# CIawevy/FreeFine

Measured on AMD Instinct MI355X. Metric: edited images/sec/GPU @512px 50-step DDIM, higher is better.
Workload: dtype bf16x3

## Files before the change

freefine_amd/_lib.py:

```python
import ctypes as C
import os

_HERE = os.path.dirname(os.path.abspath(__file__))
LIB_PATH = os.environ.get("FREEFINE_HIP_LIB") or os.path.join(_HERE, "libfreefine_hip.so")

FFN_F32, FFN_BF16, FFN_BF16X3, FFN_FP8 = 0, 1, 2, 3
IG_OUT_SILU, IG_OUT_F32, IG_GEGLU, IG_OUT_TRANSPOSED, IG_OUT_PAIR, IG_OUT_GELU, IG_OUT_RELU, IG_OUT_KV64 = 1, 2, 4, 8, 16, 32, 64, 128
IG_OUT_QGELU = 256
ELT_RELU, ELT_ADD, ELT_GELU = 0, 1, 2
ATT_MAXP, ATT_MAXB = 4, 16
ATT_HEAD_RULE, ATT_UNIFORM_SEL1, ATT_UNIFORM_SEL0, ATT_CAUSAL = 1, 2, 4, 8
NORM_SILU, NORM_OUT_PAIR = 1, 2
IMGPREP_MAX_SIDE = 4096
IMGPREP_MAX_TAPS = 2 * 3 * IMGPREP_MAX_SIDE + 1
BOX_NMS_MAX = 16384
KEEP_NONE, KEEP_SUM_LT128, KEEP_GT128 = 0, 1, 2


class IgemmDesc(C.Structure):
    _fields_ = [
        ("A", C.c_void_p), ("W", C.c_void_p), ("out", C.c_void_p),
        ("bias", C.c_void_p), ("rowbias", C.c_void_p), ("residual", C.c_void_p),
        ("M", C.c_int), ("N", C.c_int), ("K", C.c_int), ("Kpad", C.c_int),
        ("lda", C.c_int), ("ldo", C.c_int), ("ldr", C.c_int), ("ldrb", C.c_int),
        ("rows_per_batch", C.c_int),
        ("Hin", C.c_int), ("Win", C.c_int), ("Cin", C.c_int), ("Hout", C.c_int), ("Wout", C.c_int),
        ("stride", C.c_int), ("pad", C.c_int), ("upsample", C.c_int),
        ("flags", C.c_int), ("alpha", C.c_float), ("conv", C.c_int),
        ("splitk", C.c_int), ("ws", C.c_void_p), ("ws_bytes", C.c_long),
        ("a_lo", C.c_int), ("x3", C.c_int), ("f8", C.c_int), ("kv64_from", C.c_int),
    ]


class AttnEntry(C.Structure):
    _fields_ = [
        ("q_row", C.c_int), ("kv_row", C.c_int),
        ("w_const", C.c_float), ("w_slope", C.c_float),
        ("wq", C.c_void_p), ("kmask", C.c_void_p), ("qsel", C.c_void_p),
        ("flags", C.c_int), ("hr_row", C.c_int),
    ]


class AttnDesc(C.Structure):
    _fields_ = [
        ("q", C.c_void_p), ("k", C.c_void_p), ("vt", C.c_void_p), ("out", C.c_void_p), ("w_dev", C.c_void_p),
        ("Bo", C.c_int), ("S", C.c_int), ("Sk", C.c_int), ("heads", C.c_int), ("D", C.c_int),
        ("ldq", C.c_int), ("ldk", C.c_int), ("ldvt", C.c_int), ("ldo", C.c_int),
        ("scale", C.c_float), ("npass", C.c_int), ("out_pair", C.c_int), ("kv_pair", C.c_int),
        ("e", AttnEntry * (ATT_MAXP * ATT_MAXB)),
    ]


class CtrlStepDesc(C.Structure):
    _fields_ = [
        ("eps", C.c_void_p), ("x", C.c_void_p), ("noise", C.c_void_p), ("m", C.c_void_p), ("om", C.c_void_p),
        ("x_prev", C.c_void_p), ("pred_x0", C.c_void_p),
        ("c_bt", C.c_float), ("c_at", C.c_float), ("c_ap", C.c_float), ("c_dir", C.c_float),
        ("c_dirm", C.c_float * 8), ("stdv", C.c_float * 8), ("row_masked", C.c_int * 8),
        ("rows", C.c_int), ("CHW", C.c_int), ("HW", C.c_int),
    ]


class SplatXform(C.Structure):
    _fields_ = [("center", C.c_float * 3), ("translate", C.c_float * 3), ("rotate", C.c_float * 9), ("scale", C.c_float * 3),
                ("tan_half_fov", C.c_float)]


class PackDesc(C.Structure):
    _fields_ = [
        ("src", C.c_void_p), ("dst", C.c_void_p), ("src_row", C.c_int * 16),
        ("B", C.c_int), ("Cl", C.c_int), ("CP", C.c_int), ("HW", C.c_int),
    ]


class DiftDesc(C.Structure):
    _fields_ = [
        ("src", C.c_void_p), ("tgt", C.c_void_p), ("kps", C.c_void_p), ("ws", C.c_void_p), ("out_rc", C.c_void_p), ("out_cos", C.c_void_p),
        ("ws_bytes", C.c_long), ("es", C.c_long),
        ("dtype", C.c_int), ("E", C.c_int), ("C", C.c_int), ("ld", C.c_int), ("h", C.c_int), ("w", C.c_int), ("H", C.c_int), ("W", C.c_int), ("K", C.c_int),
    ]


class ResizePilDesc(C.Structure):
    _fields_ = [
        ("src", C.c_void_p), ("dst", C.c_void_p), ("scratch", C.c_void_p), ("m1", C.c_void_p), ("m2", C.c_void_p),
        ("hbounds", C.c_void_p), ("hcoef", C.c_void_p), ("vbounds", C.c_void_p), ("vcoef", C.c_void_p),
        ("B", C.c_int), ("H", C.c_int), ("W", C.c_int), ("C", C.c_int), ("oh", C.c_int), ("ow", C.c_int), ("hksize", C.c_int), ("vksize", C.c_int),
        ("y0", C.c_int), ("x0", C.c_int), ("ch", C.c_int), ("cw", C.c_int), ("rule", C.c_int),
    ]


class CoarseEditDesc(C.Structure):
    _fields_ = [
        ("src_img", C.c_void_p), ("src_mask", C.c_void_p), ("bg", C.c_void_p), ("hole_img", C.c_void_p), ("hole_mask", C.c_void_p), ("inv", C.c_void_p),
        ("final_img", C.c_void_p), ("tmask", C.c_void_p), ("trans_hole", C.c_void_p),
        ("B", C.c_int), ("H", C.c_int), ("W", C.c_int), ("mask_c", C.c_int), ("hole_mask_c", C.c_int),
    ]


_vp, _i, _f, _l = C.c_void_p, C.c_int, C.c_float, C.c_long
SYMBOLS = {
    "ffn_version": (_i, []),
    "ffn_last_error": (C.c_char_p, []),
    "ffn_device_info": (_i, [_i, C.c_char_p, _i]),
    "ffn_graph_launch": (_i, [_vp, _vp]),
    "ffn_igemm": (_i, [_vp, _i, C.POINTER(IgemmDesc)]),
    "ffn_conv3x3_n4": (_i, [_vp, _i, _vp, _vp, _vp, _vp, _i, _i, _i, _i]),
    "ffn_split_pair": (_i, [_vp, _vp, _vp, _l, _i, _i]),
    "ffn_groupnorm_f8": (_i, [_vp, _vp, _vp, _vp, _vp, _i, _i, _i, _i, _i, _f, _i, _f, _vp, _vp, _vp]),
    "ffn_attn": (_i, [_vp, _i, C.POINTER(AttnDesc)]),
    "ffn_attn_kernel_name": (_i, [_i, C.POINTER(AttnDesc), C.c_char_p, _i]),
    "ffn_igemm_tune": (_i, [_vp, _i, C.POINTER(IgemmDesc)]),
    "ffn_igemm_tune_entry_ints": (_i, []),
    "ffn_igemm_tune_export": (_i, [C.POINTER(C.c_int), _i]),
    "ffn_igemm_tune_import": (_i, [C.POINTER(C.c_int), _i]),
    "ffn_igemm_tune_stamp": (_i, []),
    "ffn_igemm_tune_clear": (_i, []),
    "ffn_igemm_tune_enable": (_i, [_i]),
    "ffn_igemm_num_configs": (_i, []),
    "ffn_igemm_force_config": (_i, [_i]),
    "ffn_igemm_kernel_name": (_i, [_i, C.POINTER(IgemmDesc), C.c_char_p, _i]),
    "ffn_attn_presplit": (_i, [_vp, _vp, _vp, _vp, _vp, _i, _i, _i, _i, _i]),
    "ffn_attn_variant": (_i, [_i, _i, C.POINTER(C.c_int), C.POINTER(C.c_int)]),
    "ffn_gn_nchunk": (_i, [_i]),
    "ffn_gn_fused": (_i, [_i, _i, _i, _i]),
    "ffn_gn_stats": (_i, [_vp, _i, _vp, _vp, _vp, _i, _i, _i, _i, _f, _vp, _vp, _vp]),
    "ffn_gn_apply": (_i, [_vp, _i, _vp, _vp, _vp, _vp, _i, _i, _i, _i]),
    "ffn_groupnorm": (_i, [_vp, _i, _vp, _vp, _vp, _vp, _i, _i, _i, _i, _f, _i, _vp, _vp, _vp]),
    "ffn_groupnorm_pair_raw": (_i, [_vp, _vp, _vp, _vp, _vp, _vp, _i, _i, _i, _i, _f, _i, _vp, _vp, _vp]),
    "ffn_layernorm": (_i, [_vp, _i, _vp, _vp, _vp, _vp, _i, _i, _f]),
    "ffn_layernorm_pair": (_i, [_vp, _vp, _vp, _vp, _vp, _i, _i, _f]),
    "ffn_softmax_rows": (_i, [_vp, _i, _vp, _vp, _l, _i, _f]),
    "ffn_pool_layernorm": (_i, [_vp, _i, _vp, _vp, _vp, _vp, _vp, _i, _i, _i, _f, _i]),
    "ffn_cosine_rows": (_i, [_vp, _vp, _vp, _vp, _i, _i, _i]),
    "ffn_cfg_masked": (_i, [_vp, _vp, _vp, _vp, _f, _vp, _l, _i]),
    "ffn_ddim_inv_step": (_i, [_vp, _vp, _vp, _f, _f, _f, _f, _vp, _vp, _l]),
    "ffn_ddim_ctrl_step": (_i, [_vp, C.POINTER(CtrlStepDesc)]),
    "ffn_pack_nchw": (_i, [_vp, _i, C.POINTER(PackDesc)]),
    "ffn_nhwc_to_nchw_f32": (_i, [_vp, _vp, _vp, _i, _i, _i, _i]),
    "ffn_concat": (_i, [_vp, _i, _vp, _vp, _vp, _l, _i, _i]),
    "ffn_timestep_embed": (_i, [_vp, _i, _vp, _vp, _vp, _i, _i, _i]),
    "ffn_transpose": (_i, [_vp, _i, _vp, _vp, _i, _i, _i, _i, _i]),
    "ffn_cast": (_i, [_vp, _i, _i, _vp, _vp, _l]),
    "ffn_eltwise": (_i, [_vp, _i, _i, _vp, _vp, _vp, _l]),
    "ffn_resize_bilinear": (_i, [_vp, _i, _vp, _vp, _i, _i, _i, _i, _i, _i, _i]),
    "ffn_splat_lift": (_i, [_vp, _vp, _vp, _vp, _i, _i, _i, _f, _f]),
    "ffn_splat_project": (_i, [_vp, _vp, _vp, _i, C.POINTER(SplatXform)]),
    "ffn_splat_bin": (_i, [_vp, _i, _vp, _i, _f, _i, _i, _vp, _vp, _vp]),
    "ffn_splat_render": (_i, [_vp, _vp, _vp, _vp, _vp, _f, _i, _i, _i, _vp, _vp, _vp]),
    "ffn_splat_ids": (_i, [_vp, _vp, _vp, _vp, _f, _i, _i, _i, _vp]),
    "ffn_splat_correspond": (_i, [_vp, _vp, _vp, _i, _i, _i, _vp, _i, _vp, _vp]),
    "ffn_geo_project": (_i, [_vp, _vp, C.POINTER(C.c_float), _f, _i, _i, _vp, _vp]),
    "ffn_splat_composite": (_i, [_vp, _vp, _vp, _vp, _vp, _f, _f, _i, _i, _i, _i, _i, _vp]),
    "ffn_mesh_cover": (_i, [_vp, _vp, _vp, _i, _i, _vp]),
    "ffn_embed_tokens": (_i, [_vp, _i, _vp, _vp, _vp, _vp, _l, _i, _i, _i]),
    "ffn_dift_match": (_i, [_vp, C.POINTER(DiftDesc)]),
    "ffn_dift_workspace_bytes": (_l, [_i, _i, _i, _i]),
    "ffn_sift_base": (_i, [_vp, _vp, _vp, _i, _i, _i]),
    "ffn_gauss_blur_f32": (_i, [_vp, _vp, _vp, _vp, _i, _i, _vp, _i]),
    "ffn_decimate2_f32": (_i, [_vp, _vp, _vp, _i, _i]),
    "ffn_sift_extrema": (_i, [_vp, _vp, _vp, _i, _i, _vp, _i, _vp, C.POINTER(C.c_int)]),
    "ffn_sift_refine_orient": (_i, [_vp, _vp, _vp, _i, _i, _i, _vp, _i, _vp]),
    "ffn_sift_describe": (_i, [_vp, _vp, _i, _i, _i, _vp, _i, _vp, _vp]),
    "ffn_knn2_u8": (_i, [_vp, _vp, _i, _vp, _i, _vp, _vp]),
    "ffn_resize_pil_bilinear_u8": (_i, [_vp, _vp, _vp, _vp, _i, _i, _i, _i, _i, _vp, _vp, _i, _vp, _vp, _i]),
    "ffn_resize_pil_u8": (_i, [_vp, C.POINTER(ResizePilDesc)]),
    "ffn_resize_taps8_u8": (_i, [_vp, _vp, _vp, _i, _i, _i, _i, _i, _i, _vp, _vp, _vp, _vp]),
    "ffn_resize_gather_u8": (_i, [_vp, _vp, _vp, _i, _i, _i, _i, _i, _i, _vp, _vp, _i]),
    "ffn_dilate_u8": (_i, [_vp, _vp, _vp, _vp, _i, _i, _i, _i, _i]),
    "ffn_mask_bbox_u8": (_i, [_vp, _vp, _vp, _i, _i, _i, _i]),
    "ffn_coarse_edit_2d": (_i, [_vp, C.POINTER(CoarseEditDesc)]),
    "ffn_vit_patch_rows": (_i, [_vp, _i, _vp, _vp, _vp, _i, _i, _i, _i, _i]),
    "ffn_vit_patch_rows_pair": (_i, [_vp, _vp, _vp, _vp, _i, _i, _i, _i, _i]),
    "ffn_sam_patch_rows": (_i, [_vp, _i, _vp, _vp, _i, _i, _i, _i, _i, _i, C.POINTER(C.c_float), C.POINTER(C.c_float)]),
    "ffn_sam_patch_rows_pair": (_i, [_vp, _vp, _vp, _i, _i, _i, _i, _i, _i, C.POINTER(C.c_float), C.POINTER(C.c_float)]),
    "ffn_hyper_masks": (_i, [_vp, _vp, _vp, _vp, _i, _i, _i, _i]),
    "ffn_upsample_bicubic": (_i, [_vp, _vp, _vp, _vp, _i, _i, _i, _i, _i]),
    "ffn_upsample_bicubic_stats": (_i, [_vp, _vp, _vp, _vp, _i, _i, _i, _i, _i, _f]),
    "ffn_box_nms": (_i, [_vp, _vp, _vp, _i, _f]),
    "ffn_image_to_nhwc": (_i, [_vp, _i, _vp, _vp, _l, _i]),
    "ffn_nhwc_to_image": (_i, [_vp, _i, _vp, _vp, _i, _i, _i]),
}

_lib = None


class FreeFineHipError(RuntimeError):
    pass


def load():
    global _lib
    if _lib is None:
        if not os.path.exists(LIB_PATH):
            raise FreeFineHipError(
                f"{LIB_PATH} not found: build it with `python -c 'import __graft_entry__ as g; g.build()'` "
                "(hipcc --offload-arch=gfx950). There is no CPU fallback for the product path.")
        import torch
        lib = C.CDLL(LIB_PATH)
        for name, (res, args) in SYMBOLS.items():
            fn = getattr(lib, name)
            fn.restype = res
            fn.argtypes = args
        _lib = lib
    return _lib


def check(rc, what=""):
    if rc != 0:
        msg = load().ffn_last_error()
        raise FreeFineHipError(f"{what} failed rc={rc}: {msg.decode() if msg else ''}")
```

freefine_amd/csrc/capi.hip:

```cpp
#include <hip/hip_runtime.h>
#include <stdarg.h>
#include <stdio.h>
#include <initializer_list>
#include <mutex>
#include <unordered_map>
#include <stdlib.h>
#include <string.h>

#include "../../include/freefine_hip.h"
#include "attention.h"
#include "attention_pp.h"
#include "attention_x.h"
#include "attention_x3.h"
#include "attention_x3p.h"
#include "attention_xx3.h"
#include "conv_small.h"
#include "elementwise.h"
#include "igemm.h"
#include "igemm_p8.h"
#include "norms.h"
#include "splat.h"

static thread_local char g_err[512] = "";
static int fail(int code, const char* fmt, ...) {
    va_list ap;
    va_start(ap, fmt);
    vsnprintf(g_err, sizeof(g_err), fmt, ap);
    va_end(ap);
    return code;
}
static int check_launch(const char* what) {
    hipError_t e = hipGetLastError();
    if (e != hipSuccess) return fail(FFN_EHIP, "%s: %s", what, hipGetErrorString(e));
    return FFN_OK;
}
#define LAUNCH(...)                  \
    do {                             \
        (void)hipGetLastError();     \
        hipLaunchKernelGGL(__VA_ARGS__); \
    } while (0)
#define REQUIRE(cond, ...) \
    do {                   \
        if (!(cond)) return fail(FFN_EINVAL, __VA_ARGS__); \
    } while (0)

static inline bool aligned16(const void* p) { return (reinterpret_cast<uintptr_t>(p) & 15) == 0; }
static inline int grid_for(long n, int per_block = 256, int cap = 4096) {
    long g = (n + per_block - 1) / per_block;
    if (g < 1) g = 1;
    if (g > cap) g = cap;
    return (int)g;
}

template <typename K>
static int set_lds(K kernel, int bytes) {
    static std::mutex mu;
    static std::unordered_map<const void*, int> done;
    if (bytes > 48 * 1024) {
        std::lock_guard<std::mutex> lk(mu);
        int& have = done[reinterpret_cast<const void*>(kernel)];
        if (have >= bytes) return FFN_OK;
        have = bytes;
        hipError_t e = hipFuncSetAttribute(reinterpret_cast<const void*>(kernel), hipFuncAttributeMaxDynamicSharedMemorySize, bytes);
        if (e != hipSuccess) return fail(FFN_EHIP, "hipFuncSetAttribute(%d): %s", bytes, hipGetErrorString(e));
    }
    return FFN_OK;
}

extern "C" int ffn_version(void) { return 14; }
extern "C" const char* ffn_last_error(void) { return g_err; }
extern "C" int ffn_device_info(int device, char* name, int name_len) {
    hipDeviceProp_t prop;
    hipError_t e = hipGetDeviceProperties(&prop, device);
    if (e != hipSuccess) return fail(FFN_EHIP, "hipGetDeviceProperties: %s", hipGetErrorString(e));
    if (name && name_len > 0) {
        strncpy(name, prop.gcnArchName, name_len - 1);
        name[name_len - 1] = 0;
    }
    return prop.multiProcessorCount;
}

extern "C" int ffn_graph_launch(void* stream, void* graph_exec) {
    REQUIRE(graph_exec, "graph_launch: null graph");
    hipError_t e = hipGraphLaunch(reinterpret_cast<hipGraphExec_t>(graph_exec), reinterpret_cast<hipStream_t>(stream));
    if (e != hipSuccess) return fail(FFN_EHIP, "hipGraphLaunch: %s", hipGetErrorString(e));
    return FFN_OK;
}

static int device_cus() {
    static const int n = [] {
        int dev = 0, v = 0;
        if (hipGetDevice(&dev) != hipSuccess || hipDeviceGetAttribute(&v, hipDeviceAttributeMultiprocessorCount, dev) != hipSuccess || v <= 0) v = 256;
        return v;
    }();
    return n;
}
static bool can_split(const ffn_igemm_desc& d) {
    return d.ws && d.splitk != 1 && !(d.flags & (FFN_IG_GEGLU | FFN_IG_OUT_TRANSPOSED | FFN_IG_OUT_KV64));
}
static void igemm_rule_for(int dtype, const ffn_igemm_desc& d, int* bm, int* bn, int* splitk) {
    const long t128 = (long)((d.M + 127) / 128) * ((d.N + 127) / 128);
    const long t12864 = (long)((d.M + 127) / 128) * ((d.N + 63) / 64);
    *splitk = 1;
    if (!d.conv && !(d.flags & FFN_IG_GEGLU) && d.M >= 128 && (!can_split(d) || t12864 >= 128)) {
        *bm = 128; *bn = 64;
    } else if (d.N > 64 && (t128 >= 256 || (can_split(d) && d.M > 512 && d.N >= 128))) {
        *bm = 128; *bn = 128;
    } else if (t12864 >= 256 || d.M >= 4096 || (can_split(d) && d.M >= 96 && d.N >= 64)) {
        *bm = 128; *bn = 64;
    } else { *bm = 64; *bn = 64; }
    if (can_split(d)) {
        const int kstage = dtype == FFN_F32 ? 32 : 64;
        const int nk = (d.K + kstage - 1) / kstage;
        const long tiles = (long)((d.M + *bm - 1) / *bm) * ((d.N + *bn - 1) / *bn);
        int s = d.splitk > 1 ? d.splitk : (tiles >= 224 ? 1 : (int)((448 + tiles - 1) / tiles));
        if (d.splitk <= 1 && s > nk / 6) s = nk / 6;
        const long per = (long)d.M * d.N * 4;
        if ((long)s * per > d.ws_bytes) s = (int)(d.ws_bytes / per);
        if (s > nk) s = nk;
        if (s < 1) s = 1;
        *splitk = s;
    }
}

enum { CFG_64x64, CFG_128x64, CFG_128x128_8, CFG_128x128_16, CFG_256x128, CFG_256x256, CFG_128x320, CFG_128x160, CFG_192x320, CFG_H_128x320, CFG_H_256x128, CFG_H_256x256, CFG_H_128x128, CFG_PP_256x320, CFG_PP_256x256, CFG_PP_192x320, CFG_PP_192x256, CFG_PP_256x128, CFG_COUNT };
struct IgCfgInfo { int bm, bn, nwm, nwn; };
static const IgCfgInfo kCfg[CFG_COUNT] = {{64, 64, 2, 2}, {128, 64, 4, 2}, {128, 128, 2, 4}, {128, 128, 4, 4},
                                          {256, 128, 4, 4}, {256, 256, 4, 4}, {128, 320, 4, 4}, {128, 160, 4, 2}, {192, 320, 3, 4},
                                          {128, 320, 4, 4}, {256, 128, 4, 4}, {256, 256, 4, 4}, {128, 128, 4, 4},
                                          {256, 320, 2, 4}, {256, 256, 2, 4}, {192, 320, 2, 4}, {192, 256, 2, 4},
                                          {256, 128, 2, 4}};
struct IgChoice { int cfg, splitk; };
struct TunedEntry { IgChoice ch; bool validated; };

static bool is_halo_cfg(int cfg) { return cfg == CFG_H_128x320 || cfg == CFG_H_256x128 || cfg == CFG_H_256x256 || cfg == CFG_H_128x128; }
static bool is_pp_cfg(int cfg) { return cfg >= CFG_PP_256x320 && cfg <= CFG_PP_256x128; }
static bool pp_ok(const ffn_igemm_desc& d, int bm, int bn, int splitk = 1) {
    const long lim = (1l << 31) - 4096;
    const int nkt = d.x3 ? d.K / 96 : d.K / 64;
    if (bn == 128 && (bm != 256 || !d.x3 || d.conv != 1 || splitk > 1 || d.N % 256 == 0 || d.N % 320 == 0 || (d.flags & (FFN_IG_GEGLU | FFN_IG_OUT_PAIR | FFN_IG_OUT_KV64 | FFN_IG_OUT_TRANSPOSED)))) return false;
    if (d.x3) {
        if (d.x3 != 2 || d.K % 96 != 0 || d.a_lo != 32) return false;
    } else if (d.K % 64 != 0) return false;
    if (nkt < 2 || d.N % bn != 0 || d.M < bm) return false;
    const int osz = d.x3 ? 4 : 2;
    if (splitk > 1) {
        if (!can_split(d) || nkt % splitk != 0 || nkt / splitk < 2 || (long)splitk * d.M * d.N * 4 > d.ws_bytes || (long)splitk * d.M * d.N * 4 >= lim) return false;
    } else {
        const int act_ok = (!d.residual && !d.x3 && !d.f8 && !(d.flags & FFN_IG_GEGLU)) ? (FFN_IG_OUT_GELU | FFN_IG_OUT_RELU) : 0;
        if ((d.alpha != 1.0f && !d.f8) || (d.flags & ~(FFN_IG_GEGLU | act_ok | (d.x3 ? (FFN_IG_OUT_F32 | FFN_IG_OUT_PAIR | FFN_IG_OUT_KV64) : 0)))) return false;
        if (d.f8 && (!d.conv || (d.flags & FFN_IG_GEGLU))) return false;
        if (d.x3 && (d.flags & FFN_IG_GEGLU) && !(d.flags & FFN_IG_OUT_PAIR)) return false;
        if ((d.flags & FFN_IG_OUT_PAIR) && !(d.flags & FFN_IG_GEGLU) && (d.N % 32 != 0 || (d.ldo / 2) % 32 != 0 || (d.flags & FFN_IG_OUT_TRANSPOSED))) return false;
        if ((d.flags & FFN_IG_GEGLU) && bn != 256) return false;
        if (d.rowbias && d.rows_per_batch < 128) return false;
    }
    long a_bytes;
    if (d.conv) {
        const int pix = d.x3 ? d.lda : d.Cin;
        const int cpt = d.x3 ? d.Cin / 32 : d.Cin / 64;
        if (d.Cin % (d.x3 ? 32 : 64) != 0 || d.K != (d.conv == 2 ? 4 : 9) * (d.x3 ? 3 : 1) * d.Cin) return false;
        if (d.x3 && d.lda != 2 * d.Cin) return false;
        if (d.conv == 2 && (d.f8 || d.stride != 1 || d.upsample)) return false;
        if ((long)cpt * 9 * cpt >= 65536) return false;
        a_bytes = (long)(d.M / (d.Hout * d.Wout)) * d.Hin * d.Win * pix * 2;
        if (2 * d.Hin + 2 >= 32768 || 2 * d.Win + 2 >= 32768) return false;
        if (a_bytes + 256l * pix * 2 >= lim) return false;
    } else {
        a_bytes = (long)d.M * d.lda * 2;
        if (a_bytes + 256l * d.lda * 2 >= lim) return false;
    }
    if ((long)d.N * d.Kpad * 2 >= lim || (long)(d.M + 256) * d.ldo * ((d.flags & FFN_IG_OUT_PAIR) ? 2 : osz) >= lim) return false;
    if (d.residual && (long)(d.M + 256) * d.ldr * osz >= lim) return false;
    return true;
}
static int halo_bytes_for(const ffn_igemm_desc& d, int bm) {
    if (!d.conv || d.stride != 1 || d.upsample || d.pad != 1 || d.Hin != d.Hout || d.Win != d.Wout) return 0;
    if (d.Cin % 64 != 0 || d.Cin > 30000 || d.K != 9 * d.Cin || d.M % bm != 0) return 0;
    const int H = d.Hin, W = d.Win;
    int tw, tr;
    if (W <= bm) {
        if (bm % W != 0 || (H * W) % bm != 0) return 0;
        tw = W; tr = bm / W;
    } else {
        if (W % bm != 0) return 0;
        tw = bm; tr = 1;
    }
    const int nq = ((tr + 2) * (tw + 2) + 7) / 8;
    if (nq > 4 * 16) return 0;
    return nq * 8 * 128;
}
static bool x3_cfg(int cfg) { return cfg == CFG_64x64 || cfg == CFG_128x64 || cfg == CFG_128x128_8 || is_pp_cfg(cfg); }
static ffn_igemm_desc x3_view(const ffn_igemm_desc& d) {
    ffn_igemm_desc v = d;
    v.x3 = d.x3 == 2 ? 2 : 1;
    v.f8 = 0;
    v.K = 3 * d.K;
    v.flags |= FFN_IG_OUT_F32;
    return v;
}
static ffn_igemm_desc f8_view(const ffn_igemm_desc& d) {
    ffn_igemm_desc v = d;
    v.f8 = 1;
    v.x3 = 0;
    v.K = d.K / 2;
    v.Cin = d.Cin / 2;
    v.Kpad = d.Kpad / 2;
    v.lda = d.lda / 2;
    return v;
}
static ffn_igemm_desc igemm_view(int dtype, const ffn_igemm_desc& d) {
    if (dtype == FFN_BF16X3) return x3_view(d);
    if (dtype == FFN_FP8) return f8_view(d);
    ffn_igemm_desc v = d;
    v.x3 = v.f8 = 0;
    return v;
}
static int pp_tile_height(const ffn_igemm_desc& d, int bn, std::initializer_list<int> heights, int min_fill4, bool trans = false) {
    long best = -1;
    int bh = 0;
    for (int h : heights) {
        if (trans ? d.M < h : !pp_ok(d, h, bn)) continue;
        const long tiles = (long)((d.M + h - 1) / h) * (d.N / bn);
        if (tiles * 4 < (long)device_cus() * min_fill4) continue;
        const long cost = ((tiles + device_cus() - 1) / device_cus()) * h;
        if (best < 0 || cost < best) { best = cost; bh = h; }
    }
    return bh;
}
static int pp_cfg(int bm, int bn) {
    for (int cfg = CFG_PP_256x320; cfg <= CFG_PP_256x128; ++cfg)
        if (kCfg[cfg].bm == bm && kCfg[cfg].bn == bn) return cfg;
    return -1;
}
static bool conv2_tile(const ffn_igemm_desc& d, int* bm, int* bn) {
    for (int n : {320, 256})
        for (int h : {256, 192})
            if (pp_tile_height(d, n, {h}, 0)) { *bm = h; *bn = n; return true; }
    return false;
}
static bool pp_trans_tile(const ffn_igemm_desc& d, int* bm, int* bn) {
    const long lim = (1l << 31) - 4096;
    *bn = d.N % 320 == 0 ? 320 : (d.N % 256 == 0 ? 256 : 0);
    if (!*bn || d.alpha != 1.0f || d.rows_per_batch % 16 != 0 || d.M % 4 != 0) return false;
    if (d.x3) {
        if (d.x3 != 2 || d.K % 96 != 0 || d.K < 192 || d.a_lo != 32) return false;
    } else if (d.K % 64 != 0 || d.K < 128) return false;
    if ((long)(d.M + 256) * d.lda * 2 >= lim || (long)d.N * d.Kpad * 2 >= lim) return false;
    if ((long)((d.M + d.rows_per_batch - 1) / d.rows_per_batch) * d.N * d.ldo * (d.x3 ? 4 : 2) >= lim) return false;
    return (*bm = pp_tile_height(d, *bn, {256, 192}, 0, true)) != 0;
}
static IgChoice rule_choice(int dtype, const ffn_igemm_desc& d) {
    int bm, bn, sk;
    igemm_rule_for(dtype, d, &bm, &bn, &sk);
    const int kstage = dtype == FFN_F32 ? 32 : 64;
// ... 65 lines not shown
            const int hb = halo_bytes_for(d, c.bm);
            if (hb <= 0 || d.splitk > 1 || 2 * hb + 2 * c.bn * 128 > 160 * 1024) continue;
            if ((cfg == CFG_H_128x320) && (d.flags & FFN_IG_GEGLU)) continue;
        }
        const bool halo = is_halo_cfg(cfg) || is_pp_cfg(cfg);
        if (is_pp_cfg(cfg)) {
            const long pt = (long)((d.M + c.bm - 1) / c.bm) * (d.N / (c.bn > 0 ? c.bn : 1));
            if (d.splitk <= 1 && pp_ok(d, c.bm, c.bn) && n < cap) out[n++] = IgChoice{cfg, 1};
            if (cfg != CFG_PP_256x128 && d.splitk != 1 && pt > 0 && pt < kPpSplitBelow && d.N % c.bn == 0) {
                const int nkt = d.x3 ? d.K / 96 : d.K / 64;
                int added = 0;
                for (int sgo = (int)((384 + pt - 1) / pt); sgo >= 2 && added < 2; --sgo) {
                    if (d.splitk > 1 && sgo != d.splitk) continue;
                    if (nkt % sgo != 0 || nkt / sgo < 2 || !pp_ok(d, c.bm, c.bn, sgo)) continue;
                    if (n < cap) out[n++] = IgChoice{cfg, sgo};
                    ++added;
                }
            }
            continue;
        }
        if (c.bm > 64 && c.bm >= 2 * d.M) continue;
        if (c.bn > 64 && c.bn >= 2 * d.N) continue;
        if (cfg == CFG_64x64 && (long)d.M * d.N > (1l << 22)) continue;
        const long tiles = (long)((d.M + c.bm - 1) / c.bm) * ((d.N + c.bn - 1) / c.bn);
        int splits[3] = {1, 0, 0};
        if (d.splitk > 1) {
            int sf = (can_split(d) && !halo) ? d.splitk : 1;
            if ((long)sf * per > d.ws_bytes) sf = (int)(d.ws_bytes / per);
            if (sf > nk) sf = nk;
            splits[0] = sf >= 2 ? sf : 1;
        } else if (can_split(d) && !halo) {
            for (int t = 0; t < 2; ++t) {
                int sgo = (int)(((t ? 512 : 256) + tiles / 2) / tiles);
                if (sgo > nk / 4) sgo = nk / 4;
                if ((long)sgo * per > d.ws_bytes) sgo = (int)(d.ws_bytes / per);
                if (sgo >= 2) splits[1 + t] = sgo;
            }
            if (splits[2] == splits[1]) splits[2] = 0;
        }
        for (int t = 0; t < 3 && n < cap; ++t) {
            if (!splits[t]) continue;
            bool dup = false;
            for (int j = 0; j < n; ++j) dup |= out[j].cfg == cfg && out[j].splitk == splits[t];
            if (!dup) out[n++] = IgChoice{cfg, splits[t]};
        }
    }
    return n;
}
static int g_force_cfg = -1;
extern "C" int ffn_igemm_num_configs(void) { return CFG_COUNT; }
extern "C" int ffn_igemm_force_config(int cfg) {
    const int prev = g_force_cfg;
    g_force_cfg = (cfg >= 0 && cfg < CFG_COUNT) ? cfg : -1;
    return prev;
}
static bool known_choice(const ffn_igemm_desc& d, IgChoice* ch) {
    IgChoice cand[40];
    if (g_force_cfg >= 0) {
        *ch = heuristic_choice(d);
        for (int i = candidates_for(d, cand, 40) - 1; i >= 0; --i)
            if (cand[i].cfg == g_force_cfg) *ch = cand[i];
        return true;
    }
    std::lock_guard<std::mutex> lk(g_tune_mu);
    auto it = g_tuned.find(tune_key(d));
    if (it == g_tuned.end()) return false;
    if (!it->second.validated) {
        const int nc = candidates_for(d, cand, 40);
        bool ok = false;
        for (int i = 0; i < nc; ++i) ok |= cand[i].cfg == it->second.ch.cfg && cand[i].splitk == it->second.ch.splitk;
        if (!ok) return g_tuned.erase(it), false;
        it->second.validated = true;
    }
    *ch = it->second.ch;
    return true;
}

enum IgKind { IG_RING, IG_HALO, IG_PP, IG_PP_TRANS };
struct IgemmPlan {
    IgKind kind;
    bool f32;
    int bm, bn, amode, nwm, nwn;
    bool swap, fastk, x3, f8;
    bool res, geglu, split;
    int splitk, halo_bytes, lds;
    bool reduce_f32;
    dim3 grid, block;
};
static int igemm_plan(int dtype, const ffn_igemm_desc& d, const IgChoice* ch, IgemmPlan* p) {
    *p = IgemmPlan{};
    p->f32 = dtype == FFN_F32;
    p->x3 = d.x3 != 0;
    p->f8 = d.f8 != 0;
    p->amode = d.conv ? AMODE_CONV3 : AMODE_DENSE;
    p->swap = !(d.flags & FFN_IG_OUT_TRANSPOSED);
    p->reduce_f32 = p->f32 || p->x3;
    p->splitk = 1;
    p->block = dim3(512);
    const bool tuned = ch != nullptr;
    IgChoice rule;
    if (!tuned && !p->f32 && pp_trans_tile(d, &p->bm, &p->bn)) {
        p->kind = IG_PP_TRANS;
    } else {
        if (!tuned) ch = &(rule = rule_choice(p->f32 ? FFN_F32 : FFN_BF16, d));
        REQUIRE(ch->cfg >= 0 && ch->cfg < CFG_COUNT, "igemm: bad configuration %d", ch->cfg);
        REQUIRE(!(p->x3 || p->f8) || x3_cfg(ch->cfg), "igemm: configuration %d is not built for split-bf16 / fp8 problems", ch->cfg);
        const IgCfgInfo& c = kCfg[ch->cfg];
        p->kind = is_halo_cfg(ch->cfg) ? IG_HALO : (is_pp_cfg(ch->cfg) ? IG_PP : IG_RING);
        p->bm = c.bm; p->bn = c.bn; p->nwm = c.nwm; p->nwn = c.nwn;
        p->splitk = ch->splitk;
        p->block = dim3(64 * c.nwm * c.nwn);
        if (!tuned && p->x3) p->nwm = p->nwn = 2, p->block = dim3(256);
    }
    const int ntm = (d.M + p->bm - 1) / p->bm, ntn = (d.N + p->bn - 1) / p->bn;
    switch (p->kind) {
    case IG_RING: {
        p->fastk = tuned && !p->x3 && !p->f8 && (d.conv ? d.Cin % 64 == 0 : d.K % 64 == 0) && (long)d.K * 2 + 256 <= (long)sizeof(g_zero_page);
        p->lds = 2 * (p->bm + p->bn) * 128;
        int gx = ntm * ntn;
        if (tuned || p->x3) {
            int per_cu = (160 * 1024) / p->lds;
            if (per_cu > 2048 / (int)p->block.x) per_cu = 2048 / (int)p->block.x;
            const int cap = (device_cus() * per_cu) / p->splitk;
            if (gx > cap && cap >= 8) gx = cap;
        }
        p->grid = dim3(gx, p->splitk);
        break;
    }
    case IG_HALO:
        p->halo_bytes = halo_bytes_for(d, p->bm);
        REQUIRE(p->halo_bytes > 0 && p->splitk == 1 && !p->x3 && !p->f8, "igemm: halo kernel not applicable");
        p->lds = 2 * p->halo_bytes + 2 * p->bn * 128;
        p->grid = dim3((d.M / p->bm) * ntn);
        break;
    case IG_PP:
        REQUIRE(pp_ok(d, p->bm, p->bn, p->splitk), "igemm: ping-pong kernel not applicable");
        p->split = p->splitk > 1;
        p->res = !p->split && d.residual;
        p->geglu = !p->split && !d.conv && (d.flags & FFN_IG_GEGLU);
        [[fallthrough]];
    case IG_PP_TRANS: {
        p->lds = 2 * (p->bm + p->bn) * 128 + 12288;
        const int nt = ntm * (d.N / p->bn) * p->splitk;
        p->grid = dim3(nt < device_cus() ? nt : device_cus());
        break;
    }
    }
    return FFN_OK;
}
template <typename K, typename... A>
static int igemm_launch(const IgemmPlan& p, K kern, hipStream_t s, A... args) {
    static const char* const what[] = {"igemm", "igemm(halo)", "igemm(ping-pong)", "igemm(ping-pong, transposed)"};
    if (int rc = set_lds(kern, p.lds)) return rc;
    LAUNCH(kern, p.grid, p.block, p.lds, s, args...);
    return check_launch(what[p.kind]);
}
template <typename T, int AMODE, bool SWAP, bool FASTK = false, bool X3 = false, bool F8 = false>
static int launch_ring(const IgemmPlan& p, hipStream_t s, const ffn_igemm_desc& d) {
#define FFN_RING(BM_, BN_, WM_, WN_) \
    if (p.bm == BM_ && p.bn == BN_ && p.nwm == WM_ && p.nwn == WN_) return igemm_launch(p, igemm_glds_kernel<T, BM_, BN_, AMODE, SWAP, 2, WM_, WN_, FASTK, X3, F8>, s, d)
    if constexpr (X3 && !SWAP) {
        FFN_RING(64, 64, 2, 2);
        FFN_RING(128, 64, 2, 2);
        FFN_RING(128, 128, 2, 2);
    } else {
        FFN_RING(64, 64, 2, 2);
        FFN_RING(128, 64, 4, 2);
        FFN_RING(128, 128, 2, 4);
        if constexpr (!X3 && !F8) FFN_RING(128, 128, 4, 4);
        if constexpr (sizeof(T) == 2 && SWAP && !X3 && !F8) {
            FFN_RING(256, 128, 4, 4);
            FFN_RING(256, 256, 4, 4);
            FFN_RING(128, 320, 4, 4);
            FFN_RING(128, 160, 4, 2);
            FFN_RING(192, 320, 3, 4);
        }
    }
#undef FFN_RING
    return fail(FFN_EINVAL, "igemm: no %d x %d tile on %d x %d waves for this problem", p.bm, p.bn, p.nwm, p.nwn);
}
template <int AMODE, bool X3 = false, bool F8 = false>
static int launch_pp(const IgemmPlan& p, hipStream_t s, const ffn_igemm_desc& d) {
    const bool trans = p.kind == IG_PP_TRANS;
#define FFN_PP(BM_, BN_, RES_, GEGLU_, SPLIT_, TRANS_)                                                                       \
    if (p.bm == BM_ && p.bn == BN_ && p.res == RES_ && p.geglu == GEGLU_ && p.split == SPLIT_ && trans == TRANS_) \
        return igemm_launch(p, igemm_pp_kernel<BM_, BN_, AMODE, RES_, GEGLU_, SPLIT_, TRANS_, X3, F8>, s, d, p.splitk)
#define FFN_PP_TILE(BM_, BN_)                                                                   \
    FFN_PP(BM_, BN_, false, false, false, false);                                               \
    FFN_PP(BM_, BN_, true, false, false, false);                                                \
    FFN_PP(BM_, BN_, false, false, true, false);                                                \
    if constexpr (AMODE == AMODE_DENSE && !F8) {                                                \
        FFN_PP(BM_, BN_, false, false, false, true);                                            \
        if constexpr (BN_ == 256) FFN_PP(BM_, BN_, false, true, false, false);                  \
    }
    FFN_PP_TILE(256, 320)
    FFN_PP_TILE(256, 256)
    FFN_PP_TILE(192, 320)
    FFN_PP_TILE(192, 256)
    if constexpr (X3 && AMODE == AMODE_CONV3) {
        FFN_PP(256, 128, false, false, false, false);
        FFN_PP(256, 128, true, false, false, false);
    }
#undef FFN_PP_TILE
#undef FFN_PP
    return fail(FFN_EINVAL, "igemm: no %d x %d ping-pong tile of this form", p.bm, p.bn);
}
static int igemm_run(hipStream_t s, int dtype, const ffn_igemm_desc& d, const IgChoice* ch) {
    IgemmPlan p;
    int rc = igemm_plan(dtype, d, ch, &p);
    if (rc) return rc;
    const bool conv = p.amode == AMODE_CONV3;
    switch (p.kind) {
    case IG_RING:
        if (p.f32) rc = conv ? launch_ring<float, AMODE_CONV3, true>(p, s, d) : (p.swap ? launch_ring<float, AMODE_DENSE, true>(p, s, d) : launch_ring<float, AMODE_DENSE, false>(p, s, d));
        else if (!p.swap) rc = p.x3 ? launch_ring<bf16, AMODE_DENSE, false, false, true>(p, s, d) : launch_ring<bf16, AMODE_DENSE, false>(p, s, d);
        else if (p.x3) rc = conv ? launch_ring<bf16, AMODE_CONV3, true, false, true>(p, s, d) : launch_ring<bf16, AMODE_DENSE, true, false, true>(p, s, d);
        else if (p.f8) rc = launch_ring<bf16, AMODE_CONV3, true, false, false, true>(p, s, d);
        else if (p.fastk) rc = conv ? launch_ring<bf16, AMODE_CONV3, true, true>(p, s, d) : launch_ring<bf16, AMODE_DENSE, true, true>(p, s, d);
        else rc = conv ? launch_ring<bf16, AMODE_CONV3, true>(p, s, d) : launch_ring<bf16, AMODE_DENSE, true>(p, s, d);
        break;
    case IG_HALO:
#define FFN_HALO(BM_, BN_) \
    if (p.bm == BM_ && p.bn == BN_) rc = igemm_launch(p, igemm_halo_kernel<bf16, BM_, BN_, 4, 4>, s, d, p.halo_bytes)
        FFN_HALO(128, 320);
        FFN_HALO(256, 128);
        FFN_HALO(256, 256);
        FFN_HALO(128, 128);
#undef FFN_HALO
        break;
    case IG_PP:
    case IG_PP_TRANS:
        if (p.x3) rc = conv ? launch_pp<AMODE_CONV3, true>(p, s, d) : launch_pp<AMODE_DENSE, true>(p, s, d);
        else if (p.f8) rc = launch_pp<AMODE_CONV3, false, true>(p, s, d);
        else rc = conv ? launch_pp<AMODE_CONV3>(p, s, d) : launch_pp<AMODE_DENSE>(p, s, d);
        break;
    }
    if (rc || p.splitk == 1) return rc;
    const dim3 grid(grid_for((long)d.M * (d.N / 4)));
    if (p.reduce_f32) LAUNCH(igemm_splitk_reduce_kernel<float>, grid, dim3(256), 0, s, d, p.splitk);
    else LAUNCH(igemm_splitk_reduce_kernel<bf16>, grid, dim3(256), 0, s, d, p.splitk);
    return check_launch("igemm_splitk_reduce");
}
static int igemm_tune_now(hipStream_t s, int dtype, const ffn_igemm_desc& d) {
    std::lock_guard<std::mutex> lk(g_tune_mu);
    IgChoice cand[40];
    const int nc = candidates_for(d, cand, 40);
    hipEvent_t e0, e1;
    if (hipEventCreate(&e0) != hipSuccess || hipEventCreate(&e1) != hipSuccess) return igemm_run(s, dtype, d, &cand[0]);
    IgChoice best = cand[0];
    float best_ms = 1e30f;
    const int reps = 3;
    for (int i = 0; i < nc; ++i) {
        int rc = igemm_run(s, dtype, d, &cand[i]);
        if (rc) continue;
        float ms = 1e30f;
        for (int round = 0; round < 2 && !rc; ++round) {
            (void)hipEventRecord(e0, s);
            for (int r = 0; r < reps && !rc; ++r) rc = igemm_run(s, dtype, d, &cand[i]);
            (void)hipEventRecord(e1, s);
            if (rc || hipEventSynchronize(e1) != hipSuccess) { rc = rc ? rc : FFN_EHIP; break; }
            float t = 0.f;
            (void)hipEventElapsedTime(&t, e0, e1);
            if (t < ms) ms = t;
        }
        if (rc) continue;
        if (ms < best_ms) { best_ms = ms; best = cand[i]; }
    }
    (void)hipEventDestroy(e0);
    (void)hipEventDestroy(e1);
    g_tuned[tune_key(d)] = TunedEntry{best, true};
    static const bool verbose = getenv("FFN_IGEMM_TUNE_VERBOSE") != nullptr;
    if (verbose)
        fprintf(stderr, "[ffn tune] %s M=%d N=%d K=%d flags=%d -> %dx%d split %d (%.1f us, %d candidates)\n", d.conv ? "conv" : "dense", d.M, d.N,
                d.K, d.flags, kCfg[best.cfg].bm, kCfg[best.cfg].bn, best.splitk, best_ms * 1e3f / reps, nc);
    return igemm_run(s, dtype, d, &best);
}
static constexpr int kTuneEntryInts = (int)(sizeof(TuneKey) / sizeof(int)) + 3;
static constexpr int kTuneStamp = 0x67780000 ^ (950 << 4) ^ ((int)sizeof(TuneKey) << 8) ^ CFG_COUNT ^ (4 << 24);
extern "C" int ffn_igemm_tune_entry_ints(void) { return kTuneEntryInts; }
extern "C" int ffn_igemm_tune_stamp(void) { return kTuneStamp; }
extern "C" int ffn_igemm_tune_clear(void) {
    std::lock_guard<std::mutex> lk(g_tune_mu);
    const int n = (int)g_tuned.size();
    g_tuned.clear();
    return n;
}
extern "C" int ffn_igemm_tune_enable(int on) {
    std::lock_guard<std::mutex> lk(g_tune_mu);
    const int prev = g_tune_runtime;
    g_tune_runtime = on ? 1 : 0;
    return prev;
}
extern "C" int ffn_igemm_tune_export(int* buf, int max_entries) {
    std::lock_guard<std::mutex> lk(g_tune_mu);
    int n = 0;
    for (const auto& kv : g_tuned) {
        if (buf && n < max_entries) {
            int* e = buf + (long)n * kTuneEntryInts;
            e[0] = kTuneStamp;
            memcpy(e + 1, &kv.first, sizeof(TuneKey));
            e[kTuneEntryInts - 2] = kv.second.ch.cfg;
            e[kTuneEntryInts - 1] = kv.second.ch.splitk;
        }
        ++n;
    }
    return n;
}
extern "C" int ffn_igemm_tune_import(const int* buf, int n_entries) {
    REQUIRE(buf || n_entries == 0, "igemm_tune_import: null buffer");
    std::lock_guard<std::mutex> lk(g_tune_mu);
    int n = 0;
    for (int i = 0; i < n_entries; ++i) {
        const int* e = buf + (long)i * kTuneEntryInts;
        if (e[0] != kTuneStamp) continue;
        TuneKey k;
        memcpy(&k, e + 1, sizeof(TuneKey));
        const IgChoice ch{e[kTuneEntryInts - 2], e[kTuneEntryInts - 1]};
        if (ch.cfg < 0 || ch.cfg >= CFG_COUNT || ch.splitk < 1) continue;
        g_tuned[k] = TunedEntry{ch, false};
        ++n;
    }
    return n;
}
static int igemm_validate(int dtype, const ffn_igemm_desc& d) {
    REQUIRE(dtype == FFN_F32 || dtype == FFN_BF16 || dtype == FFN_BF16X3 || dtype == FFN_FP8, "igemm: bad dtype %d", dtype);
    if (dtype == FFN_FP8) {
        REQUIRE(d.conv && d.Cin > 0 && d.Cin % 16 == 0 && d.K == 9 * d.Cin && d.Kpad >= d.K && d.Kpad % 16 == 0 && d.lda == d.Cin,
                "igemm(fp8): 3x3 convolutions with Cin %% 16 == 0 only (Cin=%d, K=%d, Kpad=%d, lda=%d)", d.Cin, d.K, d.Kpad, d.lda);
        REQUIRE(d.M > 0 && d.N > 0 && d.N % 4 == 0 && d.ldo % 4 == 0 && d.rows_per_batch > 0 && d.M % (d.Hout * d.Wout) == 0, "igemm(fp8): bad shape");
        REQUIRE(!(d.flags & (FFN_IG_GEGLU | FFN_IG_OUT_TRANSPOSED | FFN_IG_OUT_PAIR | FFN_IG_OUT_F32)), "igemm(fp8): plain / SiLU / residual epilogues only");
        REQUIRE(d.stride == 1 || d.stride == 2, "igemm(fp8): stride %d", d.stride);
        int ex = 0;
        REQUIRE(d.alpha > 0.f && frexpf(d.alpha, &ex) == 0.5f, "igemm(fp8): alpha must be a power of two (the un-scaling of two power-of-two operand scales)");
        if (d.residual) REQUIRE(d.ldr % 4 == 0 && d.ldr >= d.N, "igemm(fp8): ldr=%d must be a multiple of 4 and >= N=%d", d.ldr, d.N);
        REQUIRE(d.ldo >= d.N, "igemm(fp8): ldo=%d must be >= N=%d", d.ldo, d.N);
        return FFN_OK;
    }
    const int epc = dtype == FFN_F32 ? 4 : 8;
    const int kmul = dtype == FFN_BF16X3 ? (d.x3 == 2 ? 2 : 3) : 1;
    REQUIRE(d.M > 0 && d.N > 0 && d.K > 0, "igemm: empty problem M=%d N=%d K=%d", d.M, d.N, d.K);
    REQUIRE(d.Kpad >= kmul * d.K && d.Kpad % epc == 0, "igemm: Kpad=%d (row stride of W) must be >= %d x K=%d and a multiple of %d", d.Kpad, kmul, d.K, epc);
    if (dtype == FFN_BF16X3) {
        const int plane = d.conv ? d.Cin : d.K;
        if (d.x3 == 2) {
            REQUIRE(plane % 32 == 0 && d.a_lo == 32 && d.lda >= 2 * plane, "igemm: blocked split-bf16 operands need K (conv: Cin) %% 32 == 0, a_lo = 32, lda >= 2 x that (%d, a_lo=%d, lda=%d)", plane, d.a_lo, d.lda);
        } else {
            REQUIRE(d.a_lo % 8 == 0 && d.a_lo >= plane && d.a_lo + plane <= d.lda, "igemm: split-bf16 A needs planes of %d elements: a_lo=%d, lda=%d", plane, d.a_lo, d.lda);
        }
        REQUIRE(d.lda % 8 == 0, "igemm: lda=%d must be a multiple of 8", d.lda);
        REQUIRE(d.alpha == 1.0f, "igemm: split-bf16 problems take alpha = 1");
    }
    REQUIRE(d.K % epc == 0, "igemm: K=%d must be a multiple of %d", d.K, epc);
    REQUIRE(d.rows_per_batch > 0, "igemm: rows_per_batch must be > 0");
    if (d.conv) {
        REQUIRE(d.Cin % epc == 0, "igemm: Cin=%d must be a multiple of %d", d.Cin, epc);
        if (d.conv == 2) {
            REQUIRE((dtype == FFN_BF16 || dtype == FFN_BF16X3) && d.K == 4 * d.Cin && d.stride == 1 && d.upsample == 0 && d.pad >= 0 && d.pad <= 3 && d.splitk <= 1,
                    "igemm: 2x2 convolution needs FFN_BF16 / FFN_BF16X3, K = 4*Cin, stride 1, no upsample, pad in 0..3, no forced split");
            int bm, bn;
            REQUIRE(conv2_tile(igemm_view(dtype, d), &bm, &bn), "igemm: 2x2 convolution M=%d N=%d Cin=%d fits no ping-pong tile (Cin %% 64 (split-bf16: 32), N %% 256 / 320, M >= 192)", d.M, d.N, d.Cin);
        } else {
            REQUIRE(d.conv == 1, "igemm: conv=%d", d.conv);
            REQUIRE(d.K == 9 * d.Cin, "igemm: conv K=%d != 9*Cin=%d", d.K, 9 * d.Cin);
        }
        REQUIRE(d.stride == 1 || d.stride == 2, "igemm: stride %d", d.stride);
        REQUIRE(d.upsample == 0 || d.upsample == 1, "igemm: upsample %d", d.upsample);
        REQUIRE(d.M % (d.Hout * d.Wout) == 0, "igemm: M=%d not a multiple of Hout*Wout", d.M);
    } else {
        REQUIRE(d.lda % epc == 0, "igemm: lda=%d must be a multiple of %d", d.lda, epc);
    }
    if (d.flags & FFN_IG_OUT_KV64) {
        REQUIRE(dtype == FFN_BF16X3 && !d.conv && !d.residual && !d.rowbias && d.splitk <= 1 &&
                    !(d.flags & (FFN_IG_GEGLU | FFN_IG_OUT_PAIR | FFN_IG_OUT_SILU | FFN_IG_OUT_GELU | FFN_IG_OUT_RELU | FFN_IG_OUT_QGELU)),
                "igemm: FFN_IG_OUT_KV64 needs FFN_BF16X3, dense A, the plain epilogue and no forced split-K");
        if (d.flags & FFN_IG_OUT_TRANSPOSED) REQUIRE(d.rows_per_batch % 64 == 0 && d.M % d.rows_per_batch == 0 && d.ldo >= d.rows_per_batch && d.ldo % 64 == 0,
                                                     "igemm: KV64 transposed output needs rows_per_batch %% 64 == 0, whole batches, ldo %% 64 == 0 (rows_per_batch=%d, ldo=%d)", d.rows_per_batch, d.ldo);
        else REQUIRE(d.kv64_from >= 0 && d.kv64_from < d.N && d.kv64_from % 64 == 0 && d.N % 64 == 0 && d.ldo % 4 == 0,
                     "igemm: KV64 output needs kv64_from and N %% 64 == 0 (kv64_from=%d, N=%d)", d.kv64_from, d.N);
    }
    if (d.flags & FFN_IG_OUT_TRANSPOSED) {
        REQUIRE(!d.conv, "igemm: transposed output is only supported for dense A");
        REQUIRE(d.ldo % 4 == 0, "igemm: transposed ldo=%d must be a multiple of 4", d.ldo);
        REQUIRE(!(d.flags & (FFN_IG_GEGLU | FFN_IG_OUT_F32 | FFN_IG_OUT_SILU | FFN_IG_OUT_GELU | FFN_IG_OUT_RELU | FFN_IG_OUT_QGELU)) && !d.residual && !d.rowbias,
                "igemm: transposed output supports bias only");
    } else {
        REQUIRE(d.N % 4 == 0 && d.ldo % 4 == 0, "igemm: N=%d and ldo=%d must be multiples of 4", d.N, d.ldo);
        if (d.residual) REQUIRE(d.ldr % 4 == 0, "igemm: ldr=%d must be a multiple of 4", d.ldr);
        if (d.flags & FFN_IG_OUT_PAIR) {
            const int nout = (d.flags & FFN_IG_GEGLU) ? d.N / 2 : d.N;
            REQUIRE(dtype == FFN_BF16X3 && d.ldo % 16 == 0 && d.ldo / 2 >= nout, "igemm: pair output needs FFN_BF16X3, ldo %% 16 == 0, ldo/2 >= columns");
            REQUIRE(d.residual != d.out, "igemm: pair output cannot overwrite its fp32 residual");
            REQUIRE((d.ldo / 2) % 32 != 0 || nout % 32 == 0 || nout == d.ldo / 2, "igemm: blocked pair output (ldo/2 %% 32 == 0) needs whole 32-column blocks");
            REQUIRE(nout == d.ldo / 2 || (d.ldo / 2) % 32 == 0, "igemm: pair output into a wider row needs ldo/2 %% 32 == 0 (ldo=%d, columns=%d)", d.ldo, nout);
        }
        if (d.flags & FFN_IG_GEGLU) {
            REQUIRE(d.N % 64 == 0, "igemm: GEGLU needs N %% 64 == 0 (N=%d)", d.N);
            REQUIRE(!d.residual && !d.rowbias && !(d.flags & (FFN_IG_OUT_F32 | FFN_IG_OUT_SILU | FFN_IG_OUT_GELU | FFN_IG_OUT_RELU | FFN_IG_OUT_QGELU)), "igemm: GEGLU epilogue is exclusive");
        }
    }
    const int act = d.flags & (FFN_IG_OUT_SILU | FFN_IG_OUT_GELU | FFN_IG_OUT_RELU | FFN_IG_OUT_QGELU);
    REQUIRE((act & (act - 1)) == 0, "igemm: SILU / GELU / QGELU / RELU are mutually exclusive");
    REQUIRE(d.splitk >= 0, "igemm: splitk must be >= 0");
    if (!d.conv && dtype != FFN_BF16X3) REQUIRE(d.lda >= d.K, "igemm: lda=%d must be >= K=%d", d.lda, d.K);
    if (d.flags & FFN_IG_OUT_TRANSPOSED) {
        const int cols = d.rows_per_batch < d.M ? d.rows_per_batch : d.M;
        REQUIRE(d.ldo >= cols, "igemm: transposed ldo=%d must be >= the %d rows of a batch", d.ldo, cols);
    } else if (!(d.flags & FFN_IG_OUT_PAIR)) {
        const int nout = (d.flags & FFN_IG_GEGLU) ? d.N / 2 : d.N;
        REQUIRE(d.ldo >= nout, "igemm: ldo=%d must be >= the %d output columns", d.ldo, nout);
    }
    if (d.residual) REQUIRE(d.ldr >= d.N, "igemm: ldr=%d must be >= N=%d", d.ldr, d.N);
    return FFN_OK;
}
static bool tuned_family(int dtype, const ffn_igemm_desc& d) { return dtype != FFN_F32 && !(d.flags & FFN_IG_OUT_TRANSPOSED); }
extern "C" int ffn_igemm_kernel_name(int dtype, const ffn_igemm_desc* d0, char* buf, int len) {
    REQUIRE(d0 && buf && len > 0, "igemm_kernel_name: null argument");
    if (int rc = igemm_validate(dtype, *d0)) return rc;
    const ffn_igemm_desc d = igemm_view(dtype, *d0);
    const bool tuned = tuned_family(dtype, d);
    IgChoice ch;
    if (tuned && !known_choice(d, &ch)) ch = heuristic_choice(d);
    IgemmPlan p;
    if (int rc = igemm_plan(dtype, d, tuned ? &ch : nullptr, &p)) return rc;
    auto b = [](bool v) { return v ? "true" : "false"; };
    switch (p.kind) {
    case IG_RING:
        snprintf(buf, len, "void igemm_glds_kernel<%s, %d, %d, %d, %s, 2, %d, %d, %s, %s, %s>(ffn_igemm_desc)", p.f32 ? "float" : "bf16", p.bm, p.bn, p.amode,
                 b(p.swap), p.nwm, p.nwn, b(p.fastk), b(p.x3), b(p.f8));
        break;
    case IG_HALO: snprintf(buf, len, "void igemm_halo_kernel<bf16, %d, %d, %d, %d>(ffn_igemm_desc, int)", p.bm, p.bn, p.nwm, p.nwn); break;
    case IG_PP:
    case IG_PP_TRANS:
        snprintf(buf, len, "void igemm_pp_kernel<%d, %d, %d, %s, %s, %s, %s, %s, %s>(ffn_igemm_desc, int)", p.bm, p.bn, p.amode, b(p.res), b(p.geglu), b(p.split),
                 b(p.kind == IG_PP_TRANS), b(p.x3), b(p.f8));
        break;
    }
    return FFN_OK;
}
extern "C" int ffn_split_pair(void* stream, const float* src, void* dst, long rows, int C, int ld_src) {
    REQUIRE(src && dst && rows > 0 && C > 0 && C % 4 == 0 && ld_src >= C && ld_src % 4 == 0, "split_pair: bad arguments (C=%d, ld_src=%d)", C, ld_src);
    REQUIRE(aligned16(src) && aligned16(dst), "split_pair: pointers must be 16-byte aligned");
    static const int wide = [] { const char* e = getenv("FFN_PAIR8"); return e ? atoi(e) : 1; }();
    if (wide && C % 8 == 0 && ld_src % 4 == 0) LAUNCH(split_pair8_kernel, dim3(grid_for(rows * (C / 8))), dim3(256), 0, reinterpret_cast<hipStream_t>(stream), src, (bf16*)dst, rows, C, ld_src);
    else LAUNCH(split_pair_kernel, dim3(grid_for(rows * (C / 4))), dim3(256), 0, reinterpret_cast<hipStream_t>(stream), src, (bf16*)dst, rows, C, ld_src);
    return check_launch("split_pair");
}
extern "C" int ffn_conv3x3_n4(void* stream, int dtype, const void* x, const float* w, const float* bias, float* out, int B, int H, int W, int Cin) {
    REQUIRE(dtype == FFN_F32 || dtype == FFN_BF16, "conv3x3_n4: fp32 or bf16 activations");
    REQUIRE(x && w && out && aligned16(x) && aligned16(w) && aligned16(out) && (!bias || aligned16(bias)), "conv3x3_n4: null / unaligned pointer");
    REQUIRE(B > 0 && H > 0 && W > 0 && Cin > 0 && Cin % 16 == 0 && Cin <= 448, "conv3x3_n4: B=%d H=%d W=%d Cin=%d (Cin %% 16 == 0, <= 448)", B, H, W, Cin);
    hipStream_t s = reinterpret_cast<hipStream_t>(stream);
    const long npix = (long)B * H * W;
    const int lds = 36 * Cin * 4;
    dim3 grid((unsigned)((npix + 63) / 64));
    int rc;
    if (dtype == FFN_F32) {
        if ((rc = set_lds(conv3x3_n4_kernel<float>, lds))) return rc;
        LAUNCH(conv3x3_n4_kernel<float>, grid, dim3(256), lds, s, (const float*)x, w, bias, out, B, H, W, Cin);
    } else {
        if ((rc = set_lds(conv3x3_n4_kernel<bf16>, lds))) return rc;
        LAUNCH(conv3x3_n4_kernel<bf16>, grid, dim3(256), lds, s, (const bf16*)x, w, bias, out, B, H, W, Cin);
    }
    return check_launch("conv3x3_n4");
}
extern "C" int ffn_igemm(void* stream, int dtype, const ffn_igemm_desc* d0) {
    REQUIRE(d0, "igemm: null descriptor");
    if (int rc = igemm_validate(dtype, *d0)) return rc;
    if (dtype == FFN_FP8) {
        REQUIRE(d0->A && d0->W && d0->out && aligned16(d0->A) && aligned16(d0->W) && aligned16(d0->out), "igemm(fp8): A/W/out must be non-null and 16-byte aligned");
    } else {
        REQUIRE(d0->A && d0->W && d0->out, "igemm: null A/W/out");
        REQUIRE(aligned16(d0->A) && aligned16(d0->W) && aligned16(d0->out), "igemm: A/W/out must be 16-byte aligned");
    }
    if ((dtype == FFN_BF16X3 || dtype == FFN_F32) && d0->residual) REQUIRE(aligned16(d0->residual), "igemm: fp32 residual must be 16-byte aligned");
    if ((dtype == FFN_BF16 || dtype == FFN_FP8) && d0->residual)
        REQUIRE((reinterpret_cast<uintptr_t>(d0->residual) & 7) == 0, "igemm%s: bf16 residual must be 8-byte aligned", dtype == FFN_FP8 ? "(fp8)" : "");
    if (d0->ws) REQUIRE(aligned16(d0->ws) && d0->ws_bytes >= 0, "igemm%s: workspace must be 16-byte aligned", dtype == FFN_FP8 ? "(fp8)" : "");
    hipStream_t s = reinterpret_cast<hipStream_t>(stream);
    const ffn_igemm_desc d = igemm_view(dtype, *d0);
    if (!tuned_family(dtype, d)) return igemm_run(s, dtype, d, nullptr);
    IgChoice ch;
    if (!known_choice(d, &ch)) {
        hipStreamCaptureStatus cap = hipStreamCaptureStatusNone;
        (void)hipStreamIsCapturing(s, &cap);
        if (tune_enabled() && cap == hipStreamCaptureStatusNone && d.residual != d.out) return igemm_tune_now(s, dtype, d);
        ch = heuristic_choice(d);
    }
    return igemm_run(s, dtype, d, &ch);
}

extern "C" int ffn_igemm_tune(void* stream, int dtype, const ffn_igemm_desc* d) { return ffn_igemm(stream, dtype, d); }

struct AttnTile { int dp, qf, kt, occ; };
static const AttnTile kAttnTileF32[] = {{48, 2, 64, 1}, {64, 2, 64, 1}, {80, 2, 64, 1}, {160, 1, 32, 1}};
static const AttnTile kAttnTileBf16[] = {{64, 2, 64, 2}, {96, 2, 64, 1}, {160, 1, 64, 1}};
static AttnTile attn_tile(bool f32, int D) {
    const AttnTile* t = f32 ? kAttnTileF32 : kAttnTileBf16;
    const int n = f32 ? 4 : 3;
    int i = 0;
    while (i + 1 < n && D > t[i].dp) ++i;
    return t[i];
}
extern "C" int ffn_attn_variant(int dtype, int D, int* dp, int* qf) {
    REQUIRE(dp && qf, "attn_variant: null argument");
    const AttnTile t = attn_tile(dtype == FFN_F32, D);
    *dp = t.dp;
    *qf = t.qf;
    return FFN_OK;
}
static constexpr int attn_kernel_lds(int esz, int dp, int qf, int kt) {
    return 2 * (kt * (dp * esz == 128 ? 128 : dp * esz + 16) + dp * ((dp * esz == 128 && kt * esz == 128) ? 128 : kt * esz + 16)) + 4 * (dp / 16) * qf * 64 * 16 + 2 * kt;
}
static_assert(attn_kernel_lds(4, 160, 1, 32) <= 160 * 1024 && attn_kernel_lds(2, 160, 1, 64) <= 160 * 1024, "attention tile does not fit the 160 KiB LDS");

typedef void (*attn_x3w_t)(ffn_attn_desc);
extern "C" __attribute__((visibility("hidden"))) attn_x3w_t fx3w_kernel(int masks);
extern "C" __attribute__((visibility("hidden"))) int fx3w_lds_bytes(void);
// ... 699 lines not shown
    }
    return check_launch("gn_apply");
}
extern "C" int ffn_layernorm(void* stream, int dtype, const void* x, void* y, const float* gamma, const float* beta, int M, int C,
                             float eps) {
    REQUIRE(dtype == FFN_F32 || dtype == FFN_BF16, "layernorm: bad dtype");
    const int epc = dtype == FFN_F32 ? 4 : 8;
    REQUIRE(x && y && gamma && beta && C % epc == 0 && aligned16(x) && aligned16(y), "layernorm: bad arguments");
    const int cch = C / epc;
    REQUIRE(cch <= 64 * 6, "layernorm: C=%d too large", C);
    hipStream_t s = reinterpret_cast<hipStream_t>(stream);
    const int grid = (M + 3) / 4;
    if (dtype == FFN_F32) {
        if (cch <= 128) LAUNCH((layernorm_kernel<float, 2>), dim3(grid), dim3(256), 0, s, (const float*)x, (float*)y, gamma, beta, M, C, eps);
        else LAUNCH((layernorm_kernel<float, 6>), dim3(grid), dim3(256), 0, s, (const float*)x, (float*)y, gamma, beta, M, C, eps);
    } else {
        if (cch <= 128) LAUNCH((layernorm_kernel<bf16, 2>), dim3(grid), dim3(256), 0, s, (const bf16*)x, (bf16*)y, gamma, beta, M, C, eps);
        else LAUNCH((layernorm_kernel<bf16, 6>), dim3(grid), dim3(256), 0, s, (const bf16*)x, (bf16*)y, gamma, beta, M, C, eps);
    }
    return check_launch("layernorm");
}
extern "C" int ffn_layernorm_pair(void* stream, const float* x, void* y, const float* gamma, const float* beta, int M, int C, float eps) {
    REQUIRE(x && y && gamma && beta && C % 4 == 0 && aligned16(x) && aligned16(y), "layernorm_pair: bad arguments");
    const int cch = C / 4;
    REQUIRE(cch <= 64 * 6, "layernorm_pair: C=%d too large", C);
    hipStream_t s = reinterpret_cast<hipStream_t>(stream);
    const int grid = (M + 3) / 4;
    if (cch <= 128) LAUNCH((layernorm_kernel<float, 2, true>), dim3(grid), dim3(256), 0, s, x, (float*)y, gamma, beta, M, C, eps);
    else LAUNCH((layernorm_kernel<float, 6, true>), dim3(grid), dim3(256), 0, s, x, (float*)y, gamma, beta, M, C, eps);
    return check_launch("layernorm(pair)");
}
extern "C" int ffn_softmax_rows(void* stream, int dtype, const void* x, void* y, long M, int N, float scale) {
    REQUIRE(dtype == FFN_F32 || dtype == FFN_BF16, "softmax_rows: bad dtype");
    REQUIRE(x && y && M > 0 && N > 0, "softmax_rows: bad arguments");
    hipStream_t s = reinterpret_cast<hipStream_t>(stream);
    if (dtype == FFN_F32) LAUNCH(softmax_rows_kernel<float>, dim3((unsigned)M), dim3(256), 0, s, (const float*)x, (float*)y, N, scale);
    else LAUNCH(softmax_rows_kernel<bf16>, dim3((unsigned)M), dim3(256), 0, s, (const bf16*)x, (bf16*)y, N, scale);
    return check_launch("softmax_rows");
}

extern "C" int ffn_cfg_masked(void* stream, const float* eps_u, const float* eps_c, const float* mask, float cfg, float* eps, long n,
                              int HW) {
    REQUIRE(eps_u && eps_c && eps && n > 0 && HW > 0, "cfg_masked: bad arguments");
    LAUNCH(cfg_masked_kernel, dim3(grid_for(n)), dim3(256), 0, reinterpret_cast<hipStream_t>(stream), eps_u, eps_c, mask, cfg, eps, n, HW);
    return check_launch("cfg_masked");
}
extern "C" int ffn_ddim_inv_step(void* stream, const float* eps, const float* x, float c_bt, float c_at, float c_an, float c_bn,
                                 float* x_next, float* pred_x0, long n) {
    REQUIRE(eps && x && x_next && n > 0, "ddim_inv_step: bad arguments");
    LAUNCH(ddim_inv_step_kernel, dim3(grid_for(n)), dim3(256), 0, reinterpret_cast<hipStream_t>(stream), eps, x, c_bt, c_at, c_an, c_bn, x_next, pred_x0, n);
    return check_launch("ddim_inv_step");
}
extern "C" int ffn_ddim_ctrl_step(void* stream, const ffn_ctrl_step_desc* d) {
    REQUIRE(d && d->eps && d->x && d->x_prev && d->m && d->om, "ddim_ctrl_step: null pointer");
    REQUIRE(d->rows > 0 && d->rows <= 8 && d->CHW > 0 && d->HW > 0 && d->CHW % d->HW == 0, "ddim_ctrl_step: bad shape");
    LAUNCH(ddim_ctrl_step_kernel, dim3(grid_for((long)d->rows * d->CHW)), dim3(256), 0, reinterpret_cast<hipStream_t>(stream), *d);
    return check_launch("ddim_ctrl_step");
}

extern "C" int ffn_pack_nchw(void* stream, int dtype, const ffn_pack_desc* d) {
    REQUIRE(d && d->src && d->dst && d->B > 0 && d->B <= 16 && d->CP >= d->Cl, "pack_nchw: bad arguments");
    hipStream_t s = reinterpret_cast<hipStream_t>(stream);
    const long n = (long)d->B * d->HW * d->CP;
    if (dtype == FFN_F32) LAUNCH(pack_nchw_kernel<float>, dim3(grid_for(n)), dim3(256), 0, s, *d);
    else if (dtype == FFN_BF16) LAUNCH(pack_nchw_kernel<bf16>, dim3(grid_for(n)), dim3(256), 0, s, *d);
    else return fail(FFN_EINVAL, "pack_nchw: bad dtype");
    return check_launch("pack_nchw");
}
extern "C" int ffn_nhwc_to_nchw_f32(void* stream, const float* src, float* dst, int B, int HW, int C, int ld) {
    REQUIRE(src && dst && B > 0 && HW > 0 && C > 0 && ld >= C, "nhwc_to_nchw_f32: bad arguments");
    LAUNCH(nhwc_to_nchw_f32_kernel, dim3(grid_for((long)B * HW * C)), dim3(256), 0, reinterpret_cast<hipStream_t>(stream), src, dst, B, HW, C, ld);
    return check_launch("nhwc_to_nchw_f32");
}
extern "C" int ffn_concat(void* stream, int dtype, const void* a, const void* b, void* out, long rows, int C1, int C2) {
    REQUIRE(dtype == FFN_F32 || dtype == FFN_BF16, "concat: bad dtype");
    const int epc = dtype == FFN_F32 ? 4 : 8;
    REQUIRE(b && out && C1 % epc == 0 && C2 % epc == 0 && aligned16(a) && aligned16(b) && aligned16(out), "concat: bad arguments");
    hipStream_t s = reinterpret_cast<hipStream_t>(stream);
    const long n = rows * ((a ? C1 + C2 : C2) / epc);
    if (dtype == FFN_F32) LAUNCH(concat_kernel<float>, dim3(grid_for(n)), dim3(256), 0, s, (const float*)a, (const float*)b, (float*)out, rows, C1, C2);
    else LAUNCH(concat_kernel<bf16>, dim3(grid_for(n)), dim3(256), 0, s, (const bf16*)a, (const bf16*)b, (bf16*)out, rows, C1, C2);
    return check_launch("concat");
}
extern "C" int ffn_timestep_embed(void* stream, int dtype, const float* t_dev, const float* freq, void* out, int B, int half, int flip) {
    REQUIRE(t_dev && freq && out && B > 0 && half > 0, "timestep_embed: bad arguments");
    hipStream_t s = reinterpret_cast<hipStream_t>(stream);
    const int n = B * 2 * half;
    if (dtype == FFN_F32) LAUNCH(timestep_embed_kernel<float>, dim3((n + 255) / 256), dim3(256), 0, s, t_dev, freq, (float*)out, B, half, flip);
    else if (dtype == FFN_BF16) LAUNCH(timestep_embed_kernel<bf16>, dim3((n + 255) / 256), dim3(256), 0, s, t_dev, freq, (bf16*)out, B, half, flip);
    else return fail(FFN_EINVAL, "timestep_embed: bad dtype");
    return check_launch("timestep_embed");
}
extern "C" int ffn_transpose(void* stream, int dtype, const void* src, void* dst, int B, int R, int C, int ld_src, int ld_dst) {
    REQUIRE(src && dst && B > 0 && R > 0 && C > 0, "transpose: bad arguments");
    hipStream_t s = reinterpret_cast<hipStream_t>(stream);
    dim3 grid((C + 31) / 32, (R + 31) / 32, B);
    if (dtype == FFN_F32) LAUNCH(transpose_kernel<float>, grid, dim3(256), 0, s, (const float*)src, (float*)dst, R, C, ld_src, ld_dst);
    else if (dtype == FFN_BF16) LAUNCH(transpose_kernel<bf16>, grid, dim3(256), 0, s, (const bf16*)src, (bf16*)dst, R, C, ld_src, ld_dst);
    else return fail(FFN_EINVAL, "transpose: bad dtype");
    return check_launch("transpose");
}
extern "C" int ffn_cast(void* stream, int src_dtype, int dst_dtype, const void* src, void* dst, long n) {
    REQUIRE(src && dst && n > 0, "cast: bad arguments");
    hipStream_t s = reinterpret_cast<hipStream_t>(stream);
    const int grid = grid_for(n);
    if (src_dtype == FFN_F32 && dst_dtype == FFN_BF16) LAUNCH((cast_kernel<float, bf16>), dim3(grid), dim3(256), 0, s, (const float*)src, (bf16*)dst, n);
    else if (src_dtype == FFN_BF16 && dst_dtype == FFN_F32) LAUNCH((cast_kernel<bf16, float>), dim3(grid), dim3(256), 0, s, (const bf16*)src, (float*)dst, n);
    else if (src_dtype == FFN_F32 && dst_dtype == FFN_F32) LAUNCH((cast_kernel<float, float>), dim3(grid), dim3(256), 0, s, (const float*)src, (float*)dst, n);
    else if (src_dtype == FFN_BF16 && dst_dtype == FFN_BF16) LAUNCH((cast_kernel<bf16, bf16>), dim3(grid), dim3(256), 0, s, (const bf16*)src, (bf16*)dst, n);
    else return fail(FFN_EINVAL, "cast: bad dtypes %d -> %d", src_dtype, dst_dtype);
    return check_launch("cast");
}
extern "C" int ffn_image_to_nhwc(void* stream, int dtype, const uint8_t* img, void* dst, long npix, int CP) {
    REQUIRE(img && dst && npix > 0 && CP >= 3, "image_to_nhwc: bad arguments");
    hipStream_t s = reinterpret_cast<hipStream_t>(stream);
    const int grid = grid_for(npix * CP);
    if (dtype == FFN_F32) LAUNCH(image_to_nhwc_kernel<float>, dim3(grid), dim3(256), 0, s, img, (float*)dst, npix, CP);
    else if (dtype == FFN_BF16) LAUNCH(image_to_nhwc_kernel<bf16>, dim3(grid), dim3(256), 0, s, img, (bf16*)dst, npix, CP);
    else return fail(FFN_EINVAL, "image_to_nhwc: bad dtype");
    return check_launch("image_to_nhwc");
}
extern "C" int ffn_nhwc_to_image(void* stream, int dtype, const void* src, float* dst, int B, int HW, int ld) {
    REQUIRE(src && dst && B > 0 && HW > 0 && ld >= 3, "nhwc_to_image: bad arguments");
    hipStream_t s = reinterpret_cast<hipStream_t>(stream);
    const int grid = grid_for((long)B * 3 * HW);
    if (dtype == FFN_F32) LAUNCH(nhwc_to_image_kernel<float>, dim3(grid), dim3(256), 0, s, (const float*)src, dst, B, HW, ld);
    else if (dtype == FFN_BF16) LAUNCH(nhwc_to_image_kernel<bf16>, dim3(grid), dim3(256), 0, s, (const bf16*)src, dst, B, HW, ld);
    else return fail(FFN_EINVAL, "nhwc_to_image: bad dtype");
    return check_launch("nhwc_to_image");
}

extern "C" int ffn_splat_lift(void* stream, const float* depth, const int* idx, float* pts, int n, int W, int H, float fx, float fy) {
    REQUIRE(depth && idx && pts, "splat_lift: null operand");
    REQUIRE(n > 0 && W > 0 && H > 0 && (long)W * H < (1l << 31) && fx != 0.f && fy != 0.f, "splat_lift: bad shape / focal length");
    LAUNCH(splat_lift_kernel, dim3(grid_for(n)), dim3(256), 0, reinterpret_cast<hipStream_t>(stream), depth, idx, pts, n, W, H, fx, fy);
    return check_launch("splat_lift");
}
extern "C" int ffn_splat_project(void* stream, const float* pts, float* proj, int n, const ffn_splat_xform* x) {
    REQUIRE(pts && proj && x, "splat_project: null operand");
    REQUIRE(n > 0, "splat_project: empty cloud");
    SplatXform X;
    for (int i = 0; i < 3; ++i) { X.c[i] = x->center[i]; X.t[i] = x->translate[i]; X.s[i] = x->scale[i]; }
    for (int i = 0; i < 9; ++i) X.R[i] = x->rotate[i];
    REQUIRE(x->tan_half_fov > 0.f, "splat_project: tan_half_fov must be positive");
    X.inv_tan = 1.f / x->tan_half_fov;
    LAUNCH(splat_project_kernel, dim3(grid_for(n)), dim3(256), 0, reinterpret_cast<hipStream_t>(stream), pts, proj, n, X);
    return check_launch("splat_project");
}
extern "C" int ffn_splat_bin(void* stream, int fill, const float* proj, int n, float radius, int W, int H, int* counts, const int* offs, int* list) {
    REQUIRE(proj && counts, "splat_bin: null operand");
    REQUIRE(!fill || (offs && list), "splat_bin: the filling pass needs the tile offsets and the list");
    REQUIRE(n > 0 && W > 0 && H > 0 && radius > 0.f, "splat_bin: bad shape / radius");
    hipStream_t s = reinterpret_cast<hipStream_t>(stream);
    if (fill) LAUNCH(splat_bin_kernel<true>, dim3(grid_for(n)), dim3(256), 0, s, proj, n, radius, W, H, counts, offs, list);
    else LAUNCH(splat_bin_kernel<false>, dim3(grid_for(n)), dim3(256), 0, s, proj, n, radius, W, H, counts, offs, list);
    return check_launch("splat_bin");
}
extern "C" int ffn_splat_render(void* stream, const float* proj, const float* rgb, const int* offs, const int* list, float radius, int K, int W, int H,
                                float* image, int* idx_sum, uint8_t* covered) {
    REQUIRE(proj && rgb && offs && list && image && idx_sum && covered, "splat_render: null operand");
    REQUIRE(K >= 1 && K <= 32, "splat_render: points per pixel K=%d out of range (1 .. 32)", K);
    REQUIRE(W > 0 && H > 0 && radius > 0.f, "splat_render: bad shape / radius");
    hipStream_t s = reinterpret_cast<hipStream_t>(stream);
    const int tiles = ((W + 15) / 16) * ((H + 15) / 16);
    if (K <= 8) LAUNCH(splat_render_kernel<8>, dim3(tiles), dim3(256), 0, s, proj, rgb, offs, list, radius, K, W, H, image, idx_sum, covered);
    else if (K <= 16) LAUNCH(splat_render_kernel<16>, dim3(tiles), dim3(256), 0, s, proj, rgb, offs, list, radius, K, W, H, image, idx_sum, covered);
// ... 58 lines not shown
```

freefine_amd/csrc/elementwise.h:

```cpp
#pragma once
#include "common.h"
#include "../../include/freefine_hip.h"

__global__ __launch_bounds__(256) void cfg_masked_kernel(const float* __restrict__ eu, const float* __restrict__ ec,
                                                         const float* __restrict__ mask, float cfg, float* __restrict__ out,
                                                         long n, int HW) {
    for (long i = (long)blockIdx.x * 256 + threadIdx.x; i < n; i += (long)gridDim.x * 256) {
        const float d = cfg * (ec[i] - eu[i]);
        out[i] = eu[i] + (mask ? d * mask[i % HW] : d);
    }
}

__global__ __launch_bounds__(256) void ddim_inv_step_kernel(const float* __restrict__ eps, const float* __restrict__ x,
                                                            float c_bt, float c_at, float c_an, float c_bn,
                                                            float* __restrict__ x_next, float* __restrict__ pred_x0, long n) {
    for (long i = (long)blockIdx.x * 256 + threadIdx.x; i < n; i += (long)gridDim.x * 256) {
        const float e = eps[i];
        const float p0 = (x[i] - c_bt * e) / c_at;
        x_next[i] = c_an * p0 + c_bn * e;
        if (pred_x0) pred_x0[i] = p0;
    }
}

typedef ffn_ctrl_step_desc CtrlStepParams;
__global__ __launch_bounds__(256) void ddim_ctrl_step_kernel(const CtrlStepParams p) {
    const long n = (long)p.rows * p.CHW;
    for (long i = (long)blockIdx.x * 256 + threadIdx.x; i < n; i += (long)gridDim.x * 256) {
        const int b = (int)(i / p.CHW);
        const int hw = (int)(i % p.HW);
        const float e = p.eps[i];
        const float mk = p.row_masked[b] ? p.m[hw] : 1.f;
        const float omk = p.row_masked[b] ? p.om[hw] : 0.f;
        const float p0 = (p.x[i] - p.c_bt * e) / p.c_at;
        const float dirm = p.c_dirm[b] * e * mk;
        const float dir = p.c_dir * e * omk + dirm;
        float xp = p.c_ap * p0 + dir;
        if (p.noise) xp = xp + p.stdv[b] * p.noise[i] * mk;
        p.x_prev[i] = xp;
        if (p.pred_x0) p.pred_x0[i] = p0;
    }
}

typedef ffn_pack_desc PackParams;
template <typename T>
__global__ __launch_bounds__(256) void pack_nchw_kernel(const PackParams p) {
    const long n = (long)p.B * p.HW * p.CP;
    T* dst = reinterpret_cast<T*>(p.dst);
    for (long i = (long)blockIdx.x * 256 + threadIdx.x; i < n; i += (long)gridDim.x * 256) {
        const int c = (int)(i % p.CP);
        const long t = i / p.CP;
        const int hw = (int)(t % p.HW), b = (int)(t / p.HW);
        float v = 0.f;
        if (c < p.Cl) v = p.src[((long)p.src_row[b] * p.Cl + c) * p.HW + hw];
        DT<T>::st(dst + i, v);
    }
}

__global__ __launch_bounds__(256) void nhwc_to_nchw_f32_kernel(const float* __restrict__ src, float* __restrict__ dst,
                                                               int B, int HW, int C, int ld) {
    const long n = (long)B * C * HW;
    for (long i = (long)blockIdx.x * 256 + threadIdx.x; i < n; i += (long)gridDim.x * 256) {
        const int hw = (int)(i % HW);
        const long t = i / HW;
        const int c = (int)(t % C), b = (int)(t / C);
        dst[i] = src[((long)b * HW + hw) * ld + c];
    }
}

template <typename T>
__global__ __launch_bounds__(256) void concat_kernel(const T* __restrict__ a, const T* __restrict__ b, T* __restrict__ out,
                                                     long rows, int C1, int C2) {
    constexpr int EPC = DT<T>::EPC;
    const int c1 = C1 / EPC, c2 = C2 / EPC;
    const int c0 = a ? 0 : c1, ct = c1 + c2 - c0;
    const long n = rows * ct;
    for (long i = (long)blockIdx.x * 256 + threadIdx.x; i < n; i += (long)gridDim.x * 256) {
        const long r = i / ct;
        const int c = c0 + (int)(i - r * ct);
        const u32x4 v = (c < c1) ? *reinterpret_cast<const u32x4*>(a + r * C1 + c * EPC)
                                 : *reinterpret_cast<const u32x4*>(b + r * C2 + (c - c1) * EPC);
        *reinterpret_cast<u32x4*>(out + r * (C1 + C2) + c * EPC) = v;
    }
}

template <typename T>
__global__ void timestep_embed_kernel(const float* __restrict__ t_dev, const float* __restrict__ freq, T* __restrict__ out,
                                      int B, int half, int flip) {
    const int i = blockIdx.x * blockDim.x + threadIdx.x;
    if (i >= B * 2 * half) return;
    const int j = i % (2 * half);
    const float t = *t_dev;
    const int jj = j < half ? j : j - half;
    const float a = t * freq[jj];
    const bool want_cos = flip ? (j < half) : (j >= half);
    DT<T>::st(out + i, want_cos ? cosf(a) : sinf(a));
}

template <typename T>
__global__ __launch_bounds__(256) void transpose_kernel(const T* __restrict__ src, T* __restrict__ dst, int R, int C,
                                                        int ld_src, int ld_dst) {
    __shared__ float tile[32][33];
    const int b = blockIdx.z;
    const int r0 = blockIdx.y * 32, c0 = blockIdx.x * 32;
    const int tx = threadIdx.x & 31, ty = threadIdx.x >> 5;
    for (int i = ty; i < 32; i += 8) {
        const int r = r0 + i, c = c0 + tx;
        tile[i][tx] = (r < R && c < C) ? DT<T>::ld(src + ((long)b * R + r) * ld_src + c) : 0.f;
    }
    __syncthreads();
    for (int i = ty; i < 32; i += 8) {
        const int c = c0 + i, r = r0 + tx;
        if (r < R && c < C) DT<T>::st(dst + ((long)b * C + c) * ld_dst + r, tile[tx][i]);
    }
}

template <typename TS, typename TD>
__global__ __launch_bounds__(256) void cast_kernel(const TS* __restrict__ src, TD* __restrict__ dst, long n) {
    for (long i = (long)blockIdx.x * 256 + threadIdx.x; i < n; i += (long)gridDim.x * 256) DT<TD>::st(dst + i, DT<TS>::ld(src + i));
}

__global__ __launch_bounds__(256) void split_pair_kernel(const float* __restrict__ src, bf16* __restrict__ dst, long rows, int C, int ld_src) {
    const int cq = C >> 2;
    const long n = rows * cq;
    for (long i = (long)blockIdx.x * 256 + threadIdx.x; i < n; i += (long)gridDim.x * 256) {
        const long r = i / cq;
        const int c = (int)(i - r * cq) << 2;
        const f32x4 x = *reinterpret_cast<const f32x4*>(src + r * ld_src + c);
        u32x2 hi, lo;
        hi[0] = pack_bf16x2(x[0], x[1]);
        hi[1] = pack_bf16x2(x[2], x[3]);
        lo[0] = pack_bf16x2(x[0] - __uint_as_float(hi[0] << 16), x[1] - __uint_as_float(hi[0] & 0xffff0000u));
        lo[1] = pack_bf16x2(x[2] - __uint_as_float(hi[1] << 16), x[3] - __uint_as_float(hi[1] & 0xffff0000u));
        bf16* q = dst + r * 2 * C + pair_pos(c, C);
        *reinterpret_cast<u32x2*>(q) = hi;
        *reinterpret_cast<u32x2*>(q + pair_lo(C)) = lo;
    }
}

__global__ __launch_bounds__(256) void split_pair8_kernel(const float* __restrict__ src, bf16* __restrict__ dst, long rows, int C, int ld_src) {
    const int cq = C >> 3;
    const long n = rows * cq;
    const int lo_off = pair_lo(C);
    for (long i = (long)blockIdx.x * 256 + threadIdx.x; i < n; i += (long)gridDim.x * 256) {
        const long r = i / cq;
        const int c = (int)(i - r * cq) << 3;
        const f32x4 x0 = *reinterpret_cast<const f32x4*>(src + r * ld_src + c), x1 = *reinterpret_cast<const f32x4*>(src + r * ld_src + c + 4);
        const float f[8] = {x0[0], x0[1], x0[2], x0[3], x1[0], x1[1], x1[2], x1[3]};
        u32x4 hi, lo;
#pragma unroll
        for (int w = 0; w < 4; ++w) {
            hi[w] = pack_bf16x2(f[2 * w], f[2 * w + 1]);
            lo[w] = pack_bf16x2(f[2 * w] - __uint_as_float(hi[w] << 16), f[2 * w + 1] - __uint_as_float(hi[w] & 0xffff0000u));
        }
        bf16* q = dst + r * 2 * C + pair_pos(c, C);
        *reinterpret_cast<u32x4*>(q) = hi;
        *reinterpret_cast<u32x4*>(q + lo_off) = lo;
    }
}

template <typename T>
__global__ __launch_bounds__(256) void image_to_nhwc_kernel(const uint8_t* __restrict__ img, T* __restrict__ dst, long npix, int CP) {
    const long n = npix * CP;
    for (long i = (long)blockIdx.x * 256 + threadIdx.x; i < n; i += (long)gridDim.x * 256) {
        const int c = (int)(i % CP);
// ... 70 lines not shown
```

freefine_amd/csrc/igemm_p8.h:

```cpp
#pragma once
#include <type_traits>
#include "igemm.h"

#ifndef PP_PRIO
#define PP_PRIO 1
#endif
#ifndef PP_ABL
#define PP_ABL 0
#endif
#ifndef PP_TAPINNER
#define PP_TAPINNER 1
#endif
#ifdef PP_STAMP
__device__ unsigned long long pp_stamp_out[8 * 64];
#define PP_STAMP_AT(k_) do { if (blockIdx.x == 7 && s >= 24 && s < 28) { const unsigned long long t_ = __builtin_amdgcn_s_memtime(); \
    if (lane == 0) *reinterpret_cast<unsigned long long*>(smem + CV + 12288 + (wave * 64 + (s - 24) * 16 + (k_)) * 8) = t_; } } while (0)
#else
#define PP_STAMP_AT(k_) do {} while (0)
#endif
#ifdef PP_NBE
#define X3_NBE(FN_, NA_) (PP_NBE)
#else
#define X3_NBE(FN_, NA_) ((FN_) + 2 - ((FN_) + (NA_) + 1) / 2)
#endif
template <int N>
__device__ __forceinline__ void pp_wait_vmcnt() {
    if (PP_ABL != 2) asm volatile("s_waitcnt vmcnt(%0)" ::"n"(N) : "memory");
}
__device__ __forceinline__ void pp_barrier() {
    asm volatile("" ::: "memory");
    __builtin_amdgcn_s_barrier();
    asm volatile("" ::: "memory");
}

#ifdef PP_TRACE
__device__ unsigned long long pp_trace[256 * 64];
#endif
template <int BM, int BN, int AMODE, bool RES, bool GEGLU, bool SPLIT = false, bool TRANS = false, bool X3 = false, bool F8 = false>
__global__ __launch_bounds__(512) void igemm_pp_kernel(const IgemmParams p, int splitk = 1) {
    typedef bf16 T;
    constexpr int HM = BM / 2;
    constexpr int FM = HM / 16;
    constexpr int FH = FM / 2;
    constexpr int NA = BM / 64;
    constexpr int FN = BN / 64;
    constexpr int WN = BN / 4;
    constexpr int ABYTES = BM * 128, BBYTES = BN * 128, BUF = ABYTES + BBYTES;
    constexpr int CV = 2 * BUF;
    constexpr int NB1 = (FN + 1) / 2;
    constexpr int NST = (SPLIT || TRANS || X3) ? FH * FN : (GEGLU ? FH * FN / 2 : FH * ((FN + 1) / 2));
    constexpr int OSZ = (X3 && !GEGLU) ? 4 : 2;
    constexpr int OOB = (int)0x80000000;
    static_assert((BM == 256 || BM == 192) && (BN == 256 || BN == 320 || (BN == 128 && BM == 256 && X3 && AMODE == AMODE_CONV3 && !GEGLU && !SPLIT && !TRANS)), "tiles built for this kernel");
    static_assert(!GEGLU || FN % 2 == 0, "GEGLU pairs hidden / gate column blocks inside a wave");

    extern __shared__ __attribute__((aligned(16))) char smem[];

    const int tid = threadIdx.x;
    const int lane = tid & 63, wave = __builtin_amdgcn_readfirstlane(tid >> 6);
    const int wr = wave >> 2, wc = wave & 3;
    const int l15 = lane & 15, g = lane >> 4;
    const int lrow = lane >> 3, csrc = (lane & 7) ^ lrow;

    static_assert(!SPLIT || (!RES && !GEGLU), "split-K slabs carry raw accumulators: the epilogue runs in the reduce kernel");
    static_assert(!TRANS || (!RES && !GEGLU && !SPLIT && AMODE == AMODE_DENSE), "transposed output: dense A, bias only");
    static_assert(!F8 || (!X3 && !TRANS && !GEGLU), "fp8 operands: plain / residual / split-K epilogues");
    const int ntn = p.N / BN;
    const int ntm = (p.M + BM - 1) / BM;
    const int nsl = SPLIT ? splitk : 1;
    const int ntiles = ntm * ntn * nsl;
    const int G = gridDim.x;
    const int nk = (X3 ? p.K / 96 : p.K / 64) / nsl;
    const int first = __builtin_amdgcn_readfirstlane(xcd_remap(blockIdx.x, G));
    const int my_tiles = (ntiles - first + G - 1) / G;
    const int S = my_tiles * nk;

    const int PIX = X3 ? p.lda * 2 : p.Cin * 2;
    const long a_bytes = AMODE == AMODE_DENSE ? (long)p.M * p.lda * 2 : (long)(p.M / (p.Hout * p.Wout)) * p.Hin * p.Win * PIX;
    const __amdgpu_buffer_rsrc_t rsrcA = __builtin_amdgcn_make_buffer_rsrc(const_cast<void*>(p.A), 0, (int)a_bytes, 0x00020000);
    const __amdgpu_buffer_rsrc_t rsrcB = __builtin_amdgcn_make_buffer_rsrc(const_cast<void*>(p.W), 0, (int)((long)p.N * p.Kpad * 2), 0x00020000);
    const __amdgpu_buffer_rsrc_t rsrcBias = __builtin_amdgcn_make_buffer_rsrc(const_cast<float*>(p.bias), 0, p.bias ? p.N * 4 : 0, 0x00020000);
    const int nbatch = (p.M + p.rows_per_batch - 1) / p.rows_per_batch;
    const __amdgpu_buffer_rsrc_t rsrcRb =
        __builtin_amdgcn_make_buffer_rsrc(const_cast<float*>(p.rowbias), 0, p.rowbias ? ((nbatch - 1) * p.ldrb + p.N) * 4 : 0, 0x00020000);
    const long o_bytes = TRANS ? (long)((p.M + p.rows_per_batch - 1) / p.rows_per_batch) * p.N * p.ldo * OSZ : (long)p.M * p.ldo * OSZ;
    const __amdgpu_buffer_rsrc_t rsrcO = __builtin_amdgcn_make_buffer_rsrc(p.out, 0, (int)o_bytes, 0x00020000);
    const __amdgpu_buffer_rsrc_t rsrcR = __builtin_amdgcn_make_buffer_rsrc(const_cast<void*>(p.residual), 0, RES ? (int)((long)p.M * p.ldr * OSZ) : 0, 0x00020000);

    int l_tile = first, l_kt = 0;
    int l_k0 = 0;
    int a_off[NA];
    int a_yx[NA];
    int b_voff;
    const int b_step = 64 * p.Kpad * 2;
    int apiece[NA];
    if constexpr (BM == 256) {
        apiece[0] = wave; apiece[1] = 16 + wave; apiece[2] = 8 + wave; apiece[3] = 24 + wave;
    } else {
        apiece[0] = wave < 6 ? wave : wave + 6;
        apiece[1] = wave < 4 ? 14 + wave : 2 + wave;
        apiece[2] = wave < 2 ? 10 + wave : 16 + wave;
    }
    const int cpt = AMODE == AMODE_DENSE ? 1 : (X3 ? p.Cin / 32 : p.Cin / 64);
    const int cpt_rcp = (65536 + cpt - 1) / cpt;
    constexpr bool TAPIN = X3 && AMODE != AMODE_DENSE && PP_TAPINNER;
    const int ntap = p.conv == 2 ? 4 : 9;
    auto kt_split = [&](int kt, int& tap, int& c) {
        if (TAPIN) {
            c = p.conv == 2 ? (kt >> 2) : ((kt * 7282) >> 16);
            tap = kt - c * ntap;
        } else {
            tap = (kt * cpt_rcp) >> 16;
            c = kt - tap * cpt;
        }
    };
    int ka = 0, tap_ky = 0, tap_kx = 0, tap_off = 0;
    auto k_position = [&]() {
        const int kt = l_k0 + l_kt;
        if (AMODE == AMODE_DENSE) {
            ka = kt * 128;
        } else {
            int tap, c;
            kt_split(kt, tap, c);
            ka = c * 128;
            tap_ky = p.conv == 2 ? (tap >> 1) : ((tap * 21846) >> 16);
            tap_kx = tap - (p.conv == 2 ? 2 : 3) * tap_ky;
            tap_off = (tap_ky * p.Win + tap_kx) * PIX;
        }
    };
    auto w_position = [&]() {
        const int kt = l_k0 + l_kt;
        if (!TAPIN) return kt * 128;
        int tap, c;
        kt_split(kt, tap, c);
        return (tap * cpt + c) * 128;
    };
    auto prep = [&](int wtile) {
        const int tile = wtile / nsl;
        l_k0 = (wtile - tile * nsl) * nk;
        const int mt = (tile / ntn) * BM, nt = (tile % ntn) * BN;
#pragma unroll
        for (int i = 0; i < NA; ++i) {
            const int m = mt + 8 * apiece[i] + lrow;
            if (AMODE == AMODE_DENSE) {
                a_off[i] = m < p.M ? (PP_ABL == 10 ? m & 255 : m) * (p.lda * 2) + csrc * 16 : OOB;
            } else {
                const int hw = p.Hout * p.Wout;
                const int ma = PP_ABL == 10 ? (m & 255) : m;
                const int b = ma / hw, rem = ma - b * hw;
                const int yo = rem / p.Wout, xo = rem - yo * p.Wout;
                const int y0 = yo * p.stride - (p.conv == 2 ? (p.pad >> 1) : p.pad), x0 = xo * p.stride - (p.conv == 2 ? (p.pad & 1) : p.pad);
                a_off[i] = ((b * p.Hin + (y0 >> p.upsample)) * p.Win + (x0 >> p.upsample)) * PIX + csrc * 16;
                a_yx[i] = m < p.M ? ((y0 << 16) | (x0 & 0xffff)) : (int)0x80008000;
            }
        }
        b_voff = (nt + 8 * wave + lrow) * (p.Kpad * 2) + csrc * 16;
    };
    auto issue_a = [&](int i, int buf) {
        int voff = a_off[i];
        if (AMODE != AMODE_DENSE) {
            const int y0 = a_yx[i] >> 16, x0 = (int)(short)(a_yx[i] & 0xffff);
            const int yy = y0 + tap_ky, xx = x0 + tap_kx;
            const bool inb = (unsigned)yy < (unsigned)(p.Hin << p.upsample) && (unsigned)xx < (unsigned)(p.Win << p.upsample);
            int toff = tap_off;
            if (p.upsample) {
                const int dy = (tap_ky + (y0 & 1)) >> 1, dx = (tap_kx + (x0 & 1)) >> 1;
                toff = (dy * p.Win + dx) * PIX;
            }
// ... 146 lines not shown
                            acc[i][j][2] = fmaf(__uint_as_float(w1 << 16), f8_inv, c[2]);
                            acc[i][j][3] = fmaf(__uint_as_float(w1 & 0xffff0000u), f8_inv, c[3]);
                        } else {
                        acc[i][j][0] = c[0] + __uint_as_float(w0 << 16);
                        acc[i][j][1] = c[1] + __uint_as_float(w0 & 0xffff0000u);
                        acc[i][j][2] = c[2] + __uint_as_float(w1 << 16);
                        acc[i][j][3] = c[3] + __uint_as_float(w1 & 0xffff0000u);
                        }
                    } else {
                        acc[i][j] = c;
                    }
                }
            }
        }
    };
    const __amdgpu_buffer_rsrc_t rsrcWs = __builtin_amdgcn_make_buffer_rsrc(p.ws, 0, SPLIT ? (int)((long)nsl * p.M * p.N * 4) : 0, 0x00020000);
    auto store_rows = [&](int wtile, auto I0) {
        constexpr int i0 = decltype(I0)::value;
        const int tile = wtile / nsl;
        const int m0 = (tile / ntn) * BM + wr * HM, n0 = (tile % ntn) * BN + wc * WN;
        int ln = lane;
        asm volatile("" : "+v"(ln));
        const int pr = ln >> 2, pg = ln & 3;
        const int paddr = (pr + 16 * pg) * 4;
        auto perm = [&](unsigned v) { return (unsigned)__builtin_amdgcn_ds_bpermute(paddr, (int)v); };
        if constexpr (SPLIT) {
            const int slice = wtile - tile * nsl;
            const int voff = (pr * p.N + 4 * pg) * 4;
#pragma unroll
            for (int i = i0; i < i0 + FH; ++i) {
                const int vo = m0 + i * 16 + pr < p.M ? voff : OOB;
#pragma unroll
                for (int j = 0; j < FN; ++j) {
                    u32x4 w = __builtin_bit_cast(u32x4, acc[i][j]);
                    w[0] = perm(w[0]); w[1] = perm(w[1]); w[2] = perm(w[2]); w[3] = perm(w[3]);
                    __builtin_amdgcn_raw_buffer_store_b128(w, rsrcWs, vo, ((slice * p.M + m0 + i * 16) * p.N + n0 + j * 16) * 4, 0);
                }
            }
            return;
        }
        if constexpr (TRANS) {
            const int voff = (pr * p.ldo + 4 * pg) * OSZ;
#pragma unroll
            for (int i = i0; i < i0 + FH; ++i) {
                const int mb = m0 + i * 16;
                const int bb = mb / p.rows_per_batch, sb = mb - bb * p.rows_per_batch;
#pragma unroll
                for (int j = 0; j < FN; ++j) {
                    if constexpr (X3) {
                        u32x4 w4 = __builtin_bit_cast(u32x4, acc[i][j]);
                        w4[0] = perm(w4[0]); w4[1] = perm(w4[1]); w4[2] = perm(w4[2]); w4[3] = perm(w4[3]);
                        if (p.flags & FFN_IG_OUT_KV64) {
                            const float f0 = __uint_as_float(w4[0]), f1 = __uint_as_float(w4[1]), f2 = __uint_as_float(w4[2]), f3 = __uint_as_float(w4[3]);
                            u32x2 hi, lo;
                            hi[0] = pack_bf16x2(f0, f1);
                            hi[1] = pack_bf16x2(f2, f3);
                            lo[0] = pack_bf16x2(f0 - __uint_as_float(hi[0] << 16), f1 - __uint_as_float(hi[0] & 0xffff0000u));
                            lo[1] = pack_bf16x2(f2 - __uint_as_float(hi[1] << 16), f3 - __uint_as_float(hi[1] & 0xffff0000u));
                            const int vo2 = mb + 4 * pg < p.M ? (pr * p.ldo * 4 + 4 * pg * 2) : OOB;
                            const int so2 = (bb * p.N + n0 + j * 16) * p.ldo * 4 + (sb >> 6) * 256 + (sb & 63) * 2;
                            __builtin_amdgcn_raw_buffer_store_b64(hi, rsrcO, vo2, so2, 0);
                            __builtin_amdgcn_raw_buffer_store_b64(lo, rsrcO, vo2, so2 + 128, 0);
                            continue;
                        }
                        __builtin_amdgcn_raw_buffer_store_b128(w4, rsrcO, mb + 4 * pg < p.M ? voff : OOB, ((bb * p.N + n0 + j * 16) * p.ldo + sb) * 4, 0);
                        continue;
                    }
                    u32x2 w;
                    w[0] = perm(pack_bf16x2(acc[i][j][0], acc[i][j][1]));
                    w[1] = perm(pack_bf16x2(acc[i][j][2], acc[i][j][3]));
                    __builtin_amdgcn_raw_buffer_store_b64(w, rsrcO, mb + 4 * pg < p.M ? voff : OOB, ((bb * p.N + n0 + j * 16) * p.ldo + sb) * 2, 0);
                }
            }
            return;
        }
        if (PP_ABL == 4) {
#pragma unroll
            for (int i = i0; i < i0 + FH; ++i)
#pragma unroll
                for (int j = 0; j < FN; ++j) asm volatile("" ::"v"(acc[i][j]));
            return;
        }
        if constexpr (X3) {
            const int voff = (pr * p.ldo + 4 * pg) * 4;
#pragma unroll
            for (int i = i0; i < i0 + FH; ++i) {
                const int vo = m0 + i * 16 + pr < p.M ? voff : OOB;
                if constexpr (GEGLU) {
                    const int vo2 = m0 + i * 16 + pr < p.M ? (pr * p.ldo + 4 * pg) * 2 : OOB;
#pragma unroll
                    for (int j = 0; j + 1 < FN; j += 2) {
                        const f32x2_t g01 = (PP_ABL == 3 ? f32x2_t{acc[i][j + 1][0], acc[i][j + 1][1]} : gelu_erf26_2(f32x2_t{acc[i][j + 1][0], acc[i][j + 1][1]})) * f32x2_t{acc[i][j][0], acc[i][j][1]};
                        const f32x2_t g23 = (PP_ABL == 3 ? f32x2_t{acc[i][j + 1][2], acc[i][j + 1][3]} : gelu_erf26_2(f32x2_t{acc[i][j + 1][2], acc[i][j + 1][3]})) * f32x2_t{acc[i][j][2], acc[i][j][3]};
                        const float v[4] = {g01[0], g01[1], g23[0], g23[1]};
                        u32x2 hi, lo;
                        hi[0] = pack_bf16x2(v[0], v[1]);
                        hi[1] = pack_bf16x2(v[2], v[3]);
                        lo[0] = pack_bf16x2(v[0] - __uint_as_float(hi[0] << 16), v[1] - __uint_as_float(hi[0] & 0xffff0000u));
                        lo[1] = pack_bf16x2(v[2] - __uint_as_float(hi[1] << 16), v[3] - __uint_as_float(hi[1] & 0xffff0000u));
                        hi[0] = perm(hi[0]); hi[1] = perm(hi[1]); lo[0] = perm(lo[0]); lo[1] = perm(lo[1]);
                        const int so = ((m0 + i * 16) * p.ldo + n0 + (j / 2) * 16) * 2;
                        __builtin_amdgcn_raw_buffer_store_b64(hi, rsrcO, vo2, so, 0);
                        __builtin_amdgcn_raw_buffer_store_b64(lo, rsrcO, vo2, so + 64, 0);
                    }
                } else {
#pragma unroll
                    for (int j = 0; j < FN; ++j) {
                        u32x4 w = __builtin_bit_cast(u32x4, acc[i][j]);
                        w[0] = perm(w[0]); w[1] = perm(w[1]); w[2] = perm(w[2]); w[3] = perm(w[3]);
                        const int nf = n0 + j * 16;
                        if (p.flags & FFN_IG_OUT_PAIR) {
                            const float f0 = __uint_as_float(w[0]), f1 = __uint_as_float(w[1]), f2 = __uint_as_float(w[2]), f3 = __uint_as_float(w[3]);
                            u32x2 hi, lo;
                            hi[0] = pack_bf16x2(f0, f1);
                            hi[1] = pack_bf16x2(f2, f3);
                            lo[0] = pack_bf16x2(f0 - __uint_as_float(hi[0] << 16), f1 - __uint_as_float(hi[0] & 0xffff0000u));
                            lo[1] = pack_bf16x2(f2 - __uint_as_float(hi[1] << 16), f3 - __uint_as_float(hi[1] & 0xffff0000u));
                            const int vo2 = m0 + i * 16 + pr < p.M ? (pr * p.ldo + 4 * pg) * 2 : OOB;
                            const int so2 = (m0 + i * 16) * p.ldo * 2 + (nf >> 5) * 128 + (nf & 31) * 2;
                            __builtin_amdgcn_raw_buffer_store_b64(hi, rsrcO, vo2, so2, 0);
                            __builtin_amdgcn_raw_buffer_store_b64(lo, rsrcO, vo2, so2 + 64, 0);
                            continue;
                        }
                        if ((p.flags & FFN_IG_OUT_KV64) && nf >= p.kv64_from) {
                            const float f0 = __uint_as_float(w[0]), f1 = __uint_as_float(w[1]), f2 = __uint_as_float(w[2]), f3 = __uint_as_float(w[3]);
                            u32x2 hi, lo;
                            hi[0] = pack_bf16x2(f0, f1);
                            hi[1] = pack_bf16x2(f2, f3);
                            lo[0] = pack_bf16x2(f0 - __uint_as_float(hi[0] << 16), f1 - __uint_as_float(hi[0] & 0xffff0000u));
                            lo[1] = pack_bf16x2(f2 - __uint_as_float(hi[1] << 16), f3 - __uint_as_float(hi[1] & 0xffff0000u));
                            const int crel = nf - p.kv64_from;
                            const int vo2 = m0 + i * 16 + pr < p.M ? (pr * p.ldo * 4 + 4 * pg * 2) : OOB;
                            const int so2 = ((m0 + i * 16) * p.ldo + p.kv64_from) * 4 + (crel >> 6) * 256 + (crel & 63) * 2;
                            __builtin_amdgcn_raw_buffer_store_b64(hi, rsrcO, vo2, so2, 0);
                            __builtin_amdgcn_raw_buffer_store_b64(lo, rsrcO, vo2, so2 + 128, 0);
                            continue;
                        }
                        __builtin_amdgcn_raw_buffer_store_b128(w, rsrcO, vo, ((m0 + i * 16) * p.ldo + n0 + j * 16) * 4, 0);
                    }
                }
            }
            return;
        }
        if constexpr (GEGLU) {
            const int voff = (l15 * p.ldo + 4 * g) * 2;
#pragma unroll
            for (int i = i0; i < i0 + FH; ++i)
#pragma unroll
                for (int j = 0; j + 1 < FN; j += 2) {
                    const f32x2_t g01 = (PP_ABL == 3 ? f32x2_t{acc[i][j + 1][0], acc[i][j + 1][1]} : gelu_erf_fast2(f32x2_t{acc[i][j + 1][0], acc[i][j + 1][1]})) * f32x2_t{acc[i][j][0], acc[i][j][1]};
                    const f32x2_t g23 = (PP_ABL == 3 ? f32x2_t{acc[i][j + 1][2], acc[i][j + 1][3]} : gelu_erf_fast2(f32x2_t{acc[i][j + 1][2], acc[i][j + 1][3]})) * f32x2_t{acc[i][j][2], acc[i][j][3]};
                    u32x2 w;
                    w[0] = pack_bf16x2(g01[0], g01[1]);
                    w[1] = pack_bf16x2(g23[0], g23[1]);
                    __builtin_amdgcn_raw_buffer_store_b64(w, rsrcO, voff, ((m0 + i * 16) * p.ldo + n0 / 2 + (j / 2) * 16) * 2, 0);
                }
            return;
        }
        if constexpr (F8) {
#pragma unroll
            for (int i = i0; i < i0 + FH; ++i)
#pragma unroll
                for (int j = 0; j < FN; ++j) {
                    acc[i][j] *= p.alpha;
                    asm volatile("" : "+v"(acc[i][j]));
                }
            __builtin_amdgcn_sched_barrier(0);
        }
        if constexpr (!RES && !F8) {
            if (p.flags & (FFN_IG_OUT_GELU | FFN_IG_OUT_RELU)) {
                const bool gelu = p.flags & FFN_IG_OUT_GELU;
#pragma unroll
                for (int i = i0; i < i0 + FH; ++i)
#pragma unroll
                    for (int j = 0; j < FN; ++j) {
#pragma unroll
                        for (int r = 0; r < 4; ++r) acc[i][j][r] = gelu ? gelu_erf_fast(acc[i][j][r]) : fmaxf(acc[i][j][r], 0.f);
                        asm volatile("" : "+v"(acc[i][j]));
                    }
                __builtin_amdgcn_sched_barrier(0);
            }
        }
        constexpr int NOF = FN;
        const int voff8 = (pr * p.ldo + 4 * pg) * 2;
        const int voff16 = pr * p.ldo * 2 + pg * 16;
        const int paddr16 = (pr + 16 * (((pg & 1) << 1) | (pg >> 1))) * 4;
        const int ncol0 = n0;
#pragma unroll
        for (int i = i0; i < i0 + FH; ++i) {
            auto outfrag = [&](int jo, unsigned& w0, unsigned& w1) {
                w0 = pack_bf16x2(acc[i][jo][0], acc[i][jo][1]);
                w1 = pack_bf16x2(acc[i][jo][2], acc[i][jo][3]);
            };
            const int row_off = PP_ABL == 5 ? ((m0 + i * 16) & 255) * p.ldo + ncol0 % 320 : (m0 + i * 16) * p.ldo + ncol0;
#pragma unroll
            for (int jo = 0; jo + 1 < NOF; jo += 2) {
                unsigned a0, a1, b0, b1;
                outfrag(jo, a0, a1);
                outfrag(jo + 1, b0, b1);
                const auto s0 = __builtin_amdgcn_permlane16_swap(a0, b0, false, false);
                const auto s1 = __builtin_amdgcn_permlane16_swap(a1, b1, false, false);
                u32x4 v;
                v[0] = (unsigned)__builtin_amdgcn_ds_bpermute(paddr16, (int)s0[0]);
                v[1] = (unsigned)__builtin_amdgcn_ds_bpermute(paddr16, (int)s1[0]);
                v[2] = (unsigned)__builtin_amdgcn_ds_bpermute(paddr16, (int)s0[1]);
                v[3] = (unsigned)__builtin_amdgcn_ds_bpermute(paddr16, (int)s1[1]);
                if (PP_ABL == 8) asm volatile("" ::"v"(v));
                else __builtin_amdgcn_raw_buffer_store_b128(v, rsrcO, voff16, (row_off + jo * 16) * 2, 0);
            }
            if constexpr (NOF % 2 == 1) {
                unsigned a0, a1;
                outfrag(NOF - 1, a0, a1);
                u32x2 v;
                v[0] = perm(a0);
                v[1] = perm(a1);
                if (PP_ABL == 8) asm volatile("" ::"v"(v));
                else __builtin_amdgcn_raw_buffer_store_b64(v, rsrcO, voff8, (row_off + (NOF - 1) * 16) * 2, 0);
            }
        }
    };

// ... 264 lines not shown
```

freefine_amd/ops.py:

```python
import ctypes as CT
import math

import os
import threading

import torch

from . import _lib as L


def _dt(t):
    if t.dtype == torch.float32:
        return L.FFN_F32
    if t.dtype == torch.bfloat16:
        return L.FFN_BF16
    raise TypeError(f"unsupported dtype {t.dtype}")


def epc(dtype):
    return 4 if dtype == torch.float32 else 8


def kstage(dtype):
    return 8 * epc(dtype)


def _stream():
    return torch.cuda.current_stream().cuda_stream


def _p(t):
    return 0 if t is None else t.data_ptr()


_PROF = None


def profile_begin():
    global _PROF
    _PROF = []


def profile_end():
    global _PROF
    rec, _PROF = _PROF, None
    torch.cuda.synchronize()
    out = {}
    for name, flops, nbytes, s, e in rec:
        d = out.setdefault(name, dict(calls=0, total_ms=0.0, flops=0.0, bytes=0.0))
        d["calls"] += 1
        d["total_ms"] += s.elapsed_time(e)
        d["flops"] += flops
        d["bytes"] += nbytes
    return out


def _timed(name, flops, nbytes, fn):
    if _PROF is None:
        return fn()
    s, e = torch.cuda.Event(enable_timing=True), torch.cuda.Event(enable_timing=True)
    s.record()
    rc = fn()
    e.record()
    _PROF.append((name, flops, nbytes, s, e))
    return rc


def _tname(t):
    return "float" if t.dtype == torch.float32 else "bf16"


def _igemm_name(lib, dcode, d):
    buf = CT.create_string_buffer(160)
    lib.ffn_igemm_kernel_name(dcode, CT.byref(d), buf, 160)
    return buf.value.decode()


_GN_CHUNK_MB = float(os.environ.get("FFN_GN_CHUNK_MB", "0"))
_GN_RAW = os.environ.get("FFN_GN_RAW", "1") != "0"
_KV64 = os.environ.get("FFN_KV64", "1") != "0"
_ATTN_PRESPLIT = os.environ.get("FFN_ATTN_PRESPLIT", "1") != "0"


def _mark_x3(t, order=1):
    t._ffn_x3 = order
    return t


def is_x3(w):
    return bool(getattr(w, "_ffn_x3", 0))


def split_hi_lo(w):
    w = w.float()
    hi = w.to(torch.bfloat16)
    return hi, (w - hi.float()).to(torch.bfloat16)


def pack_linear(w, dtype, x3=False):
    n, k = w.shape
    if x3:
        assert k % 8 == 0, f"split-bf16 weights need K % 8 == 0 (K={k})"
        hi, lo = split_hi_lo(w)
        if k % 32 == 0:
            return _mark_x3(torch.stack([hi.reshape(n, k // 32, 32), lo.reshape(n, k // 32, 32)], dim=2).reshape(n, 2 * k).contiguous(), 2)
        return _mark_x3(torch.cat([hi, lo, hi], dim=1).contiguous(), 1)
    ks = kstage(dtype)
    kpad = (k + ks - 1) // ks * ks
    out = torch.zeros(n, kpad, dtype=dtype, device=w.device)
    out[:, :k] = w.to(dtype)
    return out


def pack_conv3x3(w, dtype, cin_pad=None, x3=False):
    cout, cin = w.shape[:2]
    cp = cin_pad or cin
    w2 = torch.zeros(cout, 3, 3, cp, dtype=torch.float32, device=w.device)
    w2[..., :cin] = w.permute(0, 2, 3, 1).float()
    if x3:
        assert cp % 8 == 0, f"split-bf16 conv weights need Cin % 8 == 0 (Cin={cp})"
        hi, lo = split_hi_lo(w2.reshape(cout, 9, cp))
        if cp % 32 == 0:
            return _mark_x3(torch.stack([hi.reshape(cout, 9, cp // 32, 32), lo.reshape(cout, 9, cp // 32, 32)], dim=3).reshape(cout, 18 * cp).contiguous(), 2)
        return _mark_x3(torch.cat([hi, lo, hi], dim=2).reshape(cout, 27 * cp).contiguous(), 1)
    return pack_linear(w2.reshape(cout, 9 * cp), dtype)


def pack_conv3x3_n4(w):
    assert w.shape[0] == 4 and w.shape[2:] == (3, 3)
    return w.float().permute(0, 2, 3, 1).reshape(4, -1).contiguous()


def conv3x3_n4_eligible(cout, cin):
    return cout == 4 and cin % 16 == 0 and cin <= 448 and os.environ.get("FFN_CONV_N4", "1") != "0"


def conv3x3_n4(x, w4, bias, B, H, W, Cin):
    lib = L.load()
    assert x.is_contiguous() and x.shape[-1] == Cin and x.dtype in (torch.float32, torch.bfloat16)
    out = torch.empty(B, H * W, 4, dtype=torch.float32, device=x.device)
    L.check(_timed("conv3x3_n4_kernel", 2.0 * B * H * W * 4 * 9 * Cin, x.element_size() * x.numel() + 16.0 * B * H * W,
                   lambda: lib.ffn_conv3x3_n4(_stream(), _dt(x), x.data_ptr(), w4.data_ptr(), _p(bias), out.data_ptr(), B, H, W, Cin)), "ffn_conv3x3_n4")
    return out


def up2x_eligible(cin, cout, rows):
    return cin % 64 == 0 and (cout % 256 == 0 or cout % 320 == 0) and rows >= 192


def pack_conv3x3_up2x(w, dtype, x3=False):
    assert dtype == torch.bfloat16 or x3
    cout, cin = w.shape[:2]
    wf = w.float()
    groups = {0: ((0,), (1, 2)), 1: ((0, 1), (2,))}
    out = torch.empty(4, cout, 2, 2, cin, dtype=torch.float32, device=w.device)
    for a in (0, 1):
        for b in (0, 1):
            for dy in (0, 1):
                for dx in (0, 1):
                    acc = torch.zeros(cout, cin, dtype=torch.float32, device=w.device)
                    for ky in groups[a][dy]:
                        for kx in groups[b][dx]:
                            acc += wf[:, :, ky, kx]
                    out[2 * a + b, :, dy, dx] = acc
    if x3:
        assert cin % 32 == 0
        hi, lo = split_hi_lo(out.reshape(4 * cout, 4, cin))
        return _mark_x3(torch.stack([hi.reshape(4 * cout, 4, cin // 32, 32), lo.reshape(4 * cout, 4, cin // 32, 32)], dim=3).reshape(4 * cout, 8 * cin).contiguous(), 2)
    return pack_linear(out.reshape(4 * cout, 4 * cin), dtype)


def conv3x3_up2x(x, w4, bias, B, Hin, Win, Cin, *, out=None):
    lib = L.load()
    cout = w4.shape[0] // 4
    x3 = is_x3(w4)
    per_img = Hin * Win * max(4 * cout * (4 if x3 else 2), Cin * (4 if x3 else 2))
    nb = max(1, ((1 << 30) - 1) // per_img)
    if B > nb:
        if out is None:
            out = torch.empty(B, 4 * Hin * Win, cout, dtype=torch.float32 if x3 else x.dtype, device=x.device)
        for b0 in range(0, B, nb):
            b1 = min(B, b0 + nb)
            conv3x3_up2x(x[b0:b1], w4, bias, b1 - b0, Hin, Win, Cin, out=out[b0:b1])
        return out
    if x3:
        xa = x if pair_width(x) is not None else split_pair(x, Cin)
        assert pair_width(xa) == Cin
        odt, dcode = torch.float32, L.FFN_BF16X3
    else:
        assert x.dtype == torch.bfloat16 and x.is_contiguous()
        xa, odt, dcode = x, x.dtype, L.FFN_BF16
    assert w4.shape[1] >= (8 if x3 else 4) * Cin
    y = torch.empty(B, Hin * Win, 4 * cout, dtype=odt, device=x.device)
    for c in range(4):
        a, b = c >> 1, c & 1
        d = L.IgemmDesc()
        d.A, d.W = xa.data_ptr(), w4.data_ptr() + c * cout * w4.stride(0) * w4.element_size()
        d.bias, d.rowbias, d.residual = _p(bias), None, None
        d.M, d.N, d.K, d.Kpad = B * Hin * Win, cout, 4 * Cin, w4.stride(0)
        d.lda, d.a_lo, d.x3 = (2 * Cin, 32, 2) if x3 else (Cin, 0, 0)
        d.rows_per_batch, d.ldrb = Hin * Win, 0
        d.out, d.ldo, d.ldr = y.data_ptr() + c * cout * y.element_size(), 4 * cout, 0
        d.Hin, d.Win, d.Cin, d.Hout, d.Wout = Hin, Win, Cin, Hin, Win
        d.stride, d.pad, d.upsample = 1, 2 * (1 - a) + (1 - b), 0
        d.flags, d.alpha, d.conv = 0, 1.0, 2
        d.splitk, d.ws, d.ws_bytes = 0, _workspace(x.device).data_ptr(), WS_BYTES
        if _PROF is None:
            L.check(lib.ffn_igemm(_stream(), dcode, CT.byref(d)), "ffn_igemm(conv 2x2)")
        else:
            L.check(_timed(_igemm_name(lib, dcode, d), 2.0 * d.M * cout * 4 * Cin, y.element_size() * (x.numel() + cout * 4 * Cin + d.M * cout),
                           lambda: lib.ffn_igemm(_stream(), dcode, CT.byref(d))), "ffn_igemm(conv 2x2)")
    if out is None:
        out = torch.empty(B, 4 * Hin * Win, cout, dtype=odt, device=x.device)
    out.view(B, Hin, 2, Win, 2, cout).copy_(y.view(B, Hin, Win, 2, 2, cout).permute(0, 1, 3, 2, 4, 5))
    return out


F8_ACT_SCALE = 16.0


def pack_conv3x3_f8(w, cin_pad=None):
    cout, cin = w.shape[:2]
    cp = cin_pad or (cin + 127) // 128 * 128
    w2 = torch.zeros(cout, 3, 3, cp, dtype=torch.float32, device=w.device)
    w2[..., :cin] = w.permute(0, 2, 3, 1).float()
    amax = float(w2.abs().max())
    k = math.floor(math.log2(448.0 / amax)) if amax > 0 else 0
    ws = 2.0 ** k
    q = (w2 * ws).clamp(-448.0, 448.0).to(torch.float8_e4m3fn).reshape(cout, 9 * cp).contiguous().view(torch.uint8)
    q._ffn_f8 = (cp, 1.0 / (ws * F8_ACT_SCALE))
    return q


def is_f8(w):
    return getattr(w, "_ffn_f8", None) is not None


def groupnorm_f8(x, gamma, beta, G, eps, Cp, silu=False, ws=None):
    lib = L.load()
    B, HW, Cc = x.shape
    assert x.dtype == torch.bfloat16
    out = torch.empty(B, HW, Cp, dtype=torch.uint8, device=x.device)
    out._ffn_f8_act = Cc
    partial, scale, shift = ws if ws is not None else gn_workspace(B, HW, Cc, x.device)
    call = lambda: lib.ffn_groupnorm_f8(_stream(), x.data_ptr(), out.data_ptr(), gamma.data_ptr(), beta.data_ptr(), B, HW, Cc, Cp, G, eps,
                                        L.NORM_SILU if silu else 0, F8_ACT_SCALE, partial.data_ptr(), scale.data_ptr(), shift.data_ptr())
    L.check(_timed("gn_partial+gn_finalize+gn_apply_f8", 0.0, x.numel() * 2.0 + out.numel(), call), "ffn_groupnorm_f8")
    return out


def pack_geglu(w, b, dtype, x3=False):
    f2, k = w.shape
    f = f2 // 2
    assert f % 16 == 0
    idx = torch.arange(f, device=w.device).reshape(f // 16, 16)
    order = torch.stack([idx, idx + f], dim=1).reshape(-1)
    wp = pack_linear(w[order], dtype, x3)
    bp = None if b is None else b[order].float().contiguous()
    return wp, bp


def _mark_pair(t, C):
    t._ffn_pair = C
    return t


def pair_width(x):
    return getattr(x, "_ffn_pair", None)


def split_pair(x, K=None):
    lib = L.load()
    assert x.dtype == torch.float32 and x.stride(-1) == 1
    K = K if K is not None else x.shape[-1]
    rows = x.numel() // x.shape[-1]
    ld = x.stride(-2) if x.ndim > 1 else x.shape[-1]
    out = torch.empty(*x.shape[:-1], 2 * K, dtype=torch.bfloat16, device=x.device)
    L.check(_timed("split_pair_kernel", 0.0, 8.0 * rows * K, lambda: lib.ffn_split_pair(_stream(), x.data_ptr(), out.data_ptr(), rows, K, ld)),
            "ffn_split_pair")
    return _mark_pair(out, K)


_WS = {}
WS_BYTES = 96 << 20


def _workspace(device):
    key = (device, torch.cuda.current_stream().cuda_stream)
    ws = _WS.get(key)
    if ws is None:
        ws = _WS[key] = torch.empty(WS_BYTES // 4, dtype=torch.float32, device=device)
    return ws

_TLS = threading.local()
# ... 405 lines not shown


def softmax_rows(x, scale=1.0, out=None):
    lib = L.load()
    N = x.shape[-1]
    M = x.numel() // N
    if out is None:
        out = torch.empty_like(x)
    L.check(_timed(f"softmax_rows_kernel<{_tname(x)}>", 0.0, 2.0 * x.numel() * x.element_size(),
                   lambda: lib.ffn_softmax_rows(_stream(), _dt(x), x.data_ptr(), out.data_ptr(), M, N, scale)), "ffn_softmax_rows")
    return out


def cfg_masked(eps_u, eps_c, mask_f, cfg, out=None):
    lib = L.load()
    if out is None:
        out = torch.empty_like(eps_u)
    HW = eps_u.shape[-1] * eps_u.shape[-2]
    L.check(_timed("cfg_masked_kernel", 0.0, 12.0 * eps_u.numel(),
                   lambda: lib.ffn_cfg_masked(_stream(), eps_u.data_ptr(), eps_c.data_ptr(), _p(mask_f), float(cfg), out.data_ptr(),
                                              eps_u.numel(), HW)), "ffn_cfg_masked")
    return out


def ddim_inv_step(eps, x, c_bt, c_at, c_an, c_bn, want_pred_x0=False):
    lib = L.load()
    x_next = torch.empty_like(x)
    p0 = torch.empty_like(x) if want_pred_x0 else None
    L.check(_timed("ddim_inv_step_kernel", 0.0, (12.0 + (4.0 if want_pred_x0 else 0.0)) * x.numel(),
                   lambda: lib.ffn_ddim_inv_step(_stream(), eps.data_ptr(), x.data_ptr(), c_bt, c_at, c_an, c_bn, x_next.data_ptr(), _p(p0),
                                                 x.numel())), "ffn_ddim_inv_step")
    return x_next, p0


def ddim_ctrl_step(eps, x, noise, m_f, om_f, c_bt, c_at, c_ap, c_dir, c_dirm, stdv, row_masked, want_pred_x0=False):
    lib = L.load()
    rows = x.shape[0]
    d = L.CtrlStepDesc()
    x_prev = torch.empty_like(x)
    p0 = torch.empty_like(x) if want_pred_x0 else None
    d.eps, d.x, d.noise, d.m, d.om = eps.data_ptr(), x.data_ptr(), _p(noise), m_f.data_ptr(), om_f.data_ptr()
    d.x_prev, d.pred_x0 = x_prev.data_ptr(), _p(p0)
    d.c_bt, d.c_at, d.c_ap, d.c_dir = c_bt, c_at, c_ap, c_dir
    for b in range(rows):
        d.c_dirm[b], d.stdv[b], d.row_masked[b] = c_dirm[b], stdv[b], int(row_masked[b])
    d.rows, d.CHW, d.HW = rows, x[0].numel(), x.shape[-1] * x.shape[-2]
    L.check(_timed("ddim_ctrl_step_kernel", 0.0, 20.0 * x.numel(), lambda: lib.ffn_ddim_ctrl_step(_stream(), CT.byref(d))), "ffn_ddim_ctrl_step")
    return x_prev, p0


def pack_nchw(src, src_rows, CP, dtype, out=None):
    lib = L.load()
    Bs, Cl, H, W = src.shape
    B = len(src_rows)
    if out is None:
        out = torch.empty(B, H * W, CP, dtype=dtype, device=src.device)
    for b0 in range(0, B, 16):
        nb = min(16, B - b0)
        d = L.PackDesc()
        d.src, d.dst = src.data_ptr(), out.data_ptr() + b0 * H * W * CP * out.element_size()
        for i in range(nb):
            d.src_row[i] = src_rows[b0 + i]
        d.B, d.Cl, d.CP, d.HW = nb, Cl, CP, H * W
        L.check(_timed(f"pack_nchw_kernel<{_tname(out)}>", 0.0, nb * H * W * (4.0 * Cl + CP * out.element_size()),
                       lambda: lib.ffn_pack_nchw(_stream(), _dt(out), CT.byref(d))), "ffn_pack_nchw")
    return out


def nhwc_to_nchw_f32(src, C_, H, W, out=None):
    lib = L.load()
    B, HW, ld = src.shape
    if out is None:
        out = torch.empty(B, C_, H, W, dtype=torch.float32, device=src.device)
    L.check(_timed("nhwc_to_nchw_f32_kernel", 0.0, 8.0 * B * HW * C_,
                   lambda: lib.ffn_nhwc_to_nchw_f32(_stream(), src.data_ptr(), out.data_ptr(), B, HW, C_, ld)), "ffn_nhwc_to_nchw_f32")
    return out


def concat(a, b, out=None):
    lib = L.load()
    C1, C2 = a.shape[-1], b.shape[-1]
    rows = a.numel() // C1
    base = getattr(a, "_ffn_cat_base", None)
    if out is None and base is not None and base.shape[-1] == C1 + C2:
        L.check(_timed(f"concat_kernel<{_tname(b)}>", 0.0, 2.0 * rows * C2 * b.element_size(),
                       lambda: lib.ffn_concat(_stream(), _dt(b), None, b.data_ptr(), base.data_ptr(), rows, C1, C2)), "ffn_concat")
        return base
    if base is not None:
        a = a.contiguous()
    if out is None:
        out = torch.empty(*a.shape[:-1], C1 + C2, dtype=a.dtype, device=a.device)
    L.check(_timed(f"concat_kernel<{_tname(a)}>", 0.0, 2.0 * rows * (C1 + C2) * a.element_size(),
                   lambda: lib.ffn_concat(_stream(), _dt(a), a.data_ptr(), b.data_ptr(), out.data_ptr(), rows, C1, C2)), "ffn_concat")
    return out


def cat_dst(shape_lead, C1, C2, dtype, device):
    base = torch.empty(*shape_lead, C1 + C2, dtype=dtype, device=device)
    view = base[..., :C1]
    view._ffn_cat_base = base
    return view


def timestep_freqs(dim, device, max_period=10000.0, shift=0.0):
    half = dim // 2
    exponent = -math.log(max_period) * torch.arange(half, dtype=torch.float32) / (half - shift)
    return torch.exp(exponent).to(device)


def timestep_embed(t_dev, freq, B, dtype, flip=True, out=None):
    lib = L.load()
    half = freq.numel()
    if out is None:
        out = torch.empty(B, 2 * half, dtype=dtype, device=freq.device)
    L.check(_timed(f"timestep_embed_kernel<{_tname(out)}>", 0.0, float(out.numel() * out.element_size()),
                   lambda: lib.ffn_timestep_embed(_stream(), _dt(out), t_dev.data_ptr(), freq.data_ptr(), out.data_ptr(), B, half,
                                                  1 if flip else 0)), "ffn_timestep_embed")
    return out


def transpose(src, ld_dst=None, out=None):
    lib = L.load()
    B, R, Cc = src.shape
    ld_dst = ld_dst or R
    if out is None:
        out = torch.zeros(B, Cc, ld_dst, dtype=src.dtype, device=src.device)
    L.check(_timed(f"transpose_kernel<{_tname(src)}>", 0.0, 2.0 * src.numel() * src.element_size(),
                   lambda: lib.ffn_transpose(_stream(), _dt(src), src.data_ptr(), out.data_ptr(), B, R, Cc, Cc, ld_dst)), "ffn_transpose")
    return out


def cast(src, dtype, out=None):
    lib = L.load()
    if out is None:
        out = torch.empty(src.shape, dtype=dtype, device=src.device)
    L.check(_timed(f"cast_kernel<{_tname(src)}, {_tname(out)}>", 0.0, float(src.numel() * (src.element_size() + out.element_size())),
                   lambda: lib.ffn_cast(_stream(), _dt(src), _dt(out), src.data_ptr(), out.data_ptr(), src.numel())), "ffn_cast")
    return out


def relu(x, out=None):
    lib = L.load()
    out = torch.empty_like(x) if out is None else out
    L.check(_timed("eltwise_kernel<relu>", 0.0, 2.0 * x.numel() * x.element_size(),
                   lambda: lib.ffn_eltwise(_stream(), _dt(x), L.ELT_RELU, x.data_ptr(), None, out.data_ptr(), x.numel())), "ffn_eltwise")
    return out


def gelu(x, out=None):
    lib = L.load()
    out = torch.empty_like(x) if out is None else out
    L.check(_timed("eltwise_kernel<gelu>", 0.0, 2.0 * x.numel() * x.element_size(),
                   lambda: lib.ffn_eltwise(_stream(), _dt(x), L.ELT_GELU, x.data_ptr(), None, out.data_ptr(), x.numel())), "ffn_eltwise")
    return out


def add(a, b, out=None):
    lib = L.load()
    assert a.shape == b.shape and a.dtype == b.dtype and a.is_contiguous() and b.is_contiguous()
    out = torch.empty_like(a) if out is None else out
    L.check(_timed("eltwise_kernel<add>", 0.0, 3.0 * a.numel() * a.element_size(),
                   lambda: lib.ffn_eltwise(_stream(), _dt(a), L.ELT_ADD, a.data_ptr(), b.data_ptr(), out.data_ptr(), a.numel())), "ffn_eltwise")
    return out


def resize_bilinear(x, B, Hin, Win, Hout, Wout, relu=False):
    lib = L.load()
    C_ = x.shape[-1]
    assert x.is_contiguous() and x.numel() == B * Hin * Win * C_
    out = torch.empty(B, Hout * Wout, C_, dtype=x.dtype, device=x.device)
    L.check(_timed("resize_bilinear_kernel", 0.0, (x.numel() + out.numel()) * x.element_size(),
                   lambda: lib.ffn_resize_bilinear(_stream(), _dt(x), x.data_ptr(), out.data_ptr(), B, Hin, Win, Hout, Wout, C_, 1 if relu else 0)),
            "ffn_resize_bilinear")
    return out


def embed_tokens(ids, table, pos, dtype, out=None):
    lib = L.load()
    assert ids.dtype == torch.int32 and ids.is_contiguous() and table.dtype == pos.dtype == torch.float32 and table.is_contiguous() and pos.is_contiguous()
    N, S = ids.shape
    V, C = table.shape
    assert pos.shape[0] >= S and pos.shape[1] == C
# ... 590 lines not shown
```

freefine_amd/unet.py:

```python
import ctypes as CT
import os
import weakref

import torch

from . import _lib as L
from . import ops
from .config import UNetConfig

_GRAPH_RAW = os.environ.get("FFN_GRAPH_RAW", "1") != "0"


class _Res:
    pass


class HipUNet:
    def __init__(self, cfg: UNetConfig, state, dtype=torch.bfloat16, device="cuda:0", x3=False, fp8_conv=False):
        assert not x3 or dtype == torch.float32, "split-bf16 mode keeps fp32 activations"
        assert not fp8_conv or dtype == torch.bfloat16, "fp8 convolutions are an option of the bf16 fast mode"
        self.x3 = bool(x3)
        self.fp8_conv = bool(fp8_conv)
        self.cfg, self.dtype, self.device = cfg, dtype, torch.device(device)
        self.in_channels = cfg.in_channels
# ... 575 lines not shown
        else:
            plan = self._self_plan(t, place, B, S, drop_ref_queries=drop is not None)
            rec = ru is not None and ru["mode"] == "record" and ru.get("kv_from") is not None and tb >= ru["kv_from"]
            img = self.x3 and not rec and (plan is None or plan["kind"] != "shared_kv") and \
                ops.kv_images_ok(C // t.heads, S, S, None if plan is None else plan["passes"], B * max(S * 2 * C, C * ldv) * 4)
            qk = ops.linear(y, t.w_qk1, None, K=C, kv64_from=C if img else None)
            vt = ops.linear(y, t.w_v1, None, K=C, rows_per_batch=S, transposed_ld=ldv, kv64_from=0 if img else None)
            if rec:
                self.last_kv.append((qk[..., C:], vt))
            a = self._attention(t, False, place, qk, qk[..., C:], vt, 2 * C, B, S, S, plan=plan, kv_images=img)
        if drop is not None:
            idx, kv_text = drop
            h, res0, B = h.index_select(0, idx), res0.index_select(0, idx), idx.shape[0]
            self._in_phase_a = True
        h = ops.linear(a, t.o1[0], t.o1[1], K=C, residual=h)
        y = ops.layernorm(h, *t.ln[1], pair=self.x3)
        q = ops.linear(y, t.w_q2, None, K=C)
        k2, vt2 = kv_text
        a = self._attention(t, True, place, q, k2, vt2, C, B, S, k2.shape[1])
        h = ops.linear(a, t.o2[0], t.o2[1], K=C, residual=h)
        y = ops.layernorm(h, *t.ln[2], pair=self.x3)
        y = ops.linear(y, t.ff1[0], t.ff1[1], K=C, geglu=True, out_pair=self.x3)
        h = ops.linear(y, t.ff2[0], t.ff2[1], K=4 * C, residual=h, out_pair=self.x3 and C % 32 == 0)
        return ops.linear(h, t.proj_out[0], t.proj_out[1], K=C, residual=res0, out=out)

    def _run(self, sample, text_kv, stop_up=None):
        cfg = self.cfg
        B, _, H, W = sample.shape
        dt = self.dtype
        ru = self._reuse
        replay = ru is not None and ru["mode"] == "replay"
        record = ru is not None and ru["mode"] == "record"
        replay_kv = ru is not None and ru["mode"] == "replay_kv"
        BB = B
        if replay:
            sample = sample.index_select(0, ru["idx_a"])
            B = sample.shape[0]
            text_kv = list(ru["text_kv_a"][:self.join_block_tb(ru["join"])]) + list(text_kv[self.join_block_tb(ru["join"]):])
        if replay_kv:
            sample = sample.index_select(0, ru["idx_a"])
            B = sample.shape[0]
            text_kv = ru["text_kv_a"]
            ru["cursor"] = 0
        if record and ru.get("kv_from") is not None:
            self.last_kv = []
        self._in_phase_a = replay
        ti = iter(text_kv)
        tb = 0
        te = ops.timestep_embed(self.t_dev, self.freq, BB, dt, flip=cfg.flip_sin_to_cos)
        e1 = ops.linear(te, self.te1[0], self.te1[1], K=self.te1[2], silu=True)
        e2 = ops.linear(e1, self.te2[0], self.te2[1], K=self.te2[2], silu=True)
        temb_all = ops.linear(e2, self.temb_w, self.temb_b, K=self.te2[0].shape[0], out_f32=True)
        temb_full = temb_all
        temb_all = temb_all[:B]
        x = ops.pack_nchw(sample, list(range(B)), self.cin_pad, dt)
        x = ops.conv3x3(x, self.conv_in[0], self.conv_in[1], B, H, W, self.cin_pad)
        skips = [(x, H, W)]
        n = len(self.down)
        for i, blk in enumerate(self.down):
            for j, r in enumerate(blk.res):
                x = self._resblock(r, x, B, H, W, temb_all)
                if blk.attn:
                    x = self._transformer_block(blk.attn[j], x, B, H, W, "down", next(ti), tb=tb)
                    tb += 1
                skips.append((x, H, W))
            if blk.down is not None:
                C = x.shape[-1]
                x = ops.conv3x3(x, blk.down[0], blk.down[1], B, H, W, C, stride=2)
                H, W = (H + 1) // 2, (W + 1) // 2
                skips.append((x, H, W))
        x = self._resblock(self.mid.res[0], x, B, H, W, temb_all)
        x = self._transformer_block(self.mid.attn[0], x, B, H, W, "mid", next(ti), tb=tb)
        tb += 1
        def cat_dst(C1, HW):
            return ops.cat_dst((B, HW), C1, skips[-1][0].shape[-1], dt, x.device) if skips else None
        x = self._resblock(self.mid.res[1], x, B, H, W, temb_all, out=cat_dst(self.mid.res[1].cout, H * W))
        for i, blk in enumerate(self.up):
            if ru is not None and ru.get("join") is not None and i == ru["join"]:
                if record:
                    self.last_boundary = [x] + [s for s, _, _ in reversed(skips)]
                if replay:
                    state = ru.get("state_run") or ru["state"]
                    assert len(state) == 1 + len(skips), (len(state), len(skips))
                    merge = lambda a, r: torch.cat([a, r.to(a.dtype)], 0).index_select(0, ru["perm"])
                    x = merge(x, state[0])
                    skips = [(merge(s, st), sh, sw) for (s, sh, sw), st in zip(skips, reversed(state[1:]))]
                    B, temb_all = BB, temb_full
                    self._in_phase_a = False
            for j, r in enumerate(blk.res):
                s, sh, sw = skips.pop()
                assert (sh, sw) == (H, W)
                x = ops.concat(x, s)
                dst = cat_dst(r.cout, H * W) if j + 1 < len(blk.res) else None
                x = self._resblock(r, x, B, H, W, temb_all, out=None if blk.attn else dst)
                if blk.attn:
                    last = replay and bool(ru.get("drop_tail")) and blk.attn[j] is self.transformers[-1]
                    drop = (ru["idx_a"], ru["text_kv_a"][-1]) if last else None
                    x = self._transformer_block(blk.attn[j], x, B, H, W, "up", next(ti), out=dst, drop=drop, tb=tb)
                    tb += 1
                    if last:
                        assert dst is None and i == len(self.up) - 1 and j == len(blk.res) - 1, "the last transformer block closes the network"
                        B, temb_all = x.shape[0], temb_full[:x.shape[0]]
            if blk.up is not None:
                C = x.shape[-1]
                if blk.up2 is not None and stop_up is None and ops.up2x_eligible(C, C, B * H * W):
                    x = ops.conv3x3_up2x(x, blk.up2, blk.up[1], B, H, W, C, out=cat_dst(C, 4 * H * W))
                else:
                    x = ops.conv3x3(x, blk.up[0], blk.up[1], B, H, W, C, upsample=True, out=cat_dst(C, 4 * H * W))
                H, W = 2 * H, 2 * W
            if stop_up is not None and i == stop_up:
                return x, H, W
        C = x.shape[-1]
        if self.conv_out_n4 is not None:
            x = ops.groupnorm(x, self.norm_out[0], self.norm_out[1], cfg.norm_num_groups, cfg.norm_eps, silu=True)
            eps = ops.conv3x3_n4(x, self.conv_out_n4, self.conv_out[1], B, H, W, C)
        else:
            x = self._gn(x, self.norm_out, cfg.norm_eps, True)
            eps = ops.conv3x3(x, self.conv_out[0], self.conv_out[1], B, H, W, C, out_f32=True)
        eps = ops.nhwc_to_nchw_f32(eps, cfg.out_channels, H, W)
        self._in_phase_a = False
        if B != BB:
            eps = torch.zeros(BB, *eps.shape[1:], dtype=eps.dtype, device=eps.device).index_copy_(0, ru["idx_a"], eps)
        return eps
```

include/freefine_hip.h:

```cpp
#ifndef FREEFINE_HIP_H
#define FREEFINE_HIP_H
#include <stdint.h>
#ifdef __cplusplus
extern "C" {
#endif

enum { FFN_F32 = 0, FFN_BF16 = 1, FFN_BF16X3 = 2 ,
       FFN_FP8 = 3  };
enum { FFN_OK = 0, FFN_EINVAL = -22, FFN_ENOSYS = -38, FFN_EHIP = -5, FFN_ENOSPC = -28 };

int ffn_version(void);
const char* ffn_last_error(void);
int ffn_device_info(int device, char* name, int name_len);
int ffn_graph_launch(void* stream, void* graph_exec);

enum {
    FFN_IG_OUT_SILU = 1 << 0,
    FFN_IG_OUT_F32 = 1 << 1,
    FFN_IG_GEGLU = 1 << 2,
    FFN_IG_OUT_TRANSPOSED = 1 << 3,
    FFN_IG_OUT_PAIR = 1 << 4,
    FFN_IG_OUT_GELU = 1 << 5,
    FFN_IG_OUT_KV64 = 1 << 7,
    FFN_IG_OUT_RELU = 1 << 6,
    FFN_IG_OUT_QGELU = 1 << 8
};
typedef struct ffn_igemm_desc {
    const void* A;
    const void* W;
    void* out;
    const float* bias;
    const float* rowbias;
    const void* residual;
    int M, N, K, Kpad;
    int lda, ldo, ldr, ldrb;
    int rows_per_batch;
    int Hin, Win, Cin, Hout, Wout, stride, pad, upsample;
    int flags;
    float alpha;
    int conv;
    int splitk;
    void* ws;
    long ws_bytes;
    int a_lo;
    int x3;
    int f8;
    int kv64_from;
} ffn_igemm_desc;
int ffn_igemm(void* stream, int dtype, const ffn_igemm_desc* d);
int ffn_split_pair(void* stream, const float* src, void* dst, long rows, int C, int ld_src);
int ffn_conv3x3_n4(void* stream, int dtype, const void* x, const float* w, const float* bias, float* out, int B, int H, int W, int Cin);
int ffn_groupnorm_f8(void* stream, const void* x_bf16, void* y_e4m3, const float* gamma, const float* beta, int B, int HW, int C, int Cp,
                     int G, float eps, int silu, float qscale, float* partial_ws, float* scale, float* shift);
int ffn_igemm_tune(void* stream, int dtype, const ffn_igemm_desc* d);
int ffn_igemm_tune_entry_ints(void);
int ffn_igemm_tune_export(int* buf, int max_entries);
int ffn_igemm_tune_import(const int* buf, int n_entries);
int ffn_igemm_tune_clear(void);
int ffn_igemm_tune_enable(int on);
int ffn_igemm_tune_stamp(void);
int ffn_igemm_num_configs(void);
int ffn_igemm_force_config(int cfg);
int ffn_igemm_kernel_name(int dtype, const ffn_igemm_desc* d, char* buf, int len);

#define FFN_ATT_MAXP 4
#define FFN_ATT_MAXB 16
enum { FFN_ATT_HEAD_RULE = 1, FFN_ATT_UNIFORM_SEL1 = 2, FFN_ATT_UNIFORM_SEL0 = 4,
       FFN_ATT_CAUSAL = 8  };
typedef struct ffn_attn_entry {
    int q_row, kv_row;
    float w_const, w_slope;
    const float* wq;
    const uint8_t* kmask;
    const uint8_t* qsel;
    int flags;
    int hr_row;
} ffn_attn_entry;
typedef struct ffn_attn_desc {
    const void* q;
    const void* k;
    const void* vt;
    void* out;
    const float* w_dev;
    int Bo, S, Sk, heads, D;
    int ldq, ldk, ldvt, ldo;
    float scale;
    int npass;
    int out_pair;
    int kv_pair;
    ffn_attn_entry e[FFN_ATT_MAXP * FFN_ATT_MAXB];
} ffn_attn_desc;
int ffn_attn(void* stream, int dtype, const ffn_attn_desc* d);
int ffn_attn_presplit(void* stream, const float* k, const float* vt, void* k_pair, void* vt_pair, int rows, int Sk, int heads, int ldk, int ldvt);
int ffn_attn_variant(int dtype, int D, int* dp, int* qf);
int ffn_attn_kernel_name(int dtype, const ffn_attn_desc* d, char* buf, int len);

enum { FFN_ELT_RELU = 0, FFN_ELT_ADD = 1, FFN_ELT_GELU = 2 };
int ffn_eltwise(void* stream, int dtype, int op, const void* a, const void* b, void* y, long n);
int ffn_resize_bilinear(void* stream, int dtype, const void* x, void* y, int B, int Hin, int Win, int Hout, int Wout, int C, int relu);

typedef struct ffn_splat_xform {
    float center[3], translate[3], rotate[9] , scale[3];
    float tan_half_fov;
} ffn_splat_xform;
int ffn_splat_lift(void* stream, const float* depth, const int* idx, float* pts, int n, int W, int H, float fx, float fy);
int ffn_splat_project(void* stream, const float* pts, float* proj, int n, const ffn_splat_xform* x);
int ffn_splat_bin(void* stream, int fill, const float* proj, int n, float radius, int W, int H, int* counts, const int* offs, int* list);
int ffn_splat_render(void* stream, const float* proj, const float* rgb, const int* offs, const int* list, float radius, int K, int W, int H,
                     float* image, int* idx_sum, uint8_t* covered);
int ffn_splat_ids(void* stream, const float* proj, const int* offs, const int* list, float radius, int K, int W, int H, int* ids);
int ffn_splat_correspond(void* stream, const float* proj, const int* idx, int n, int W, int H, const int* ids, int K, float* map, uint8_t* visible);

int ffn_geo_project(void* stream, const float* depth, const float* pose, float focal, int H, int W, float* tcoords, float* proj);
int ffn_splat_composite(void* stream, const float* proj, const float* feat, const int* offs, const int* list, float radius, float tau, int K,
                        int C, int H, int W, int round_half, float* out);
int ffn_mesh_cover(void* stream, const float* tcoords, const uint8_t* mask, int H, int W, uint8_t* cover);

enum { FFN_NORM_SILU = 1, FFN_NORM_OUT_PAIR = 2 };
int ffn_gn_nchunk(int HW);
int ffn_gn_fused(int B, int HW, int C, int G);
int ffn_gn_stats(void* stream, int dtype, const void* x, const float* gamma, const float* beta, int B, int HW, int C, int G,
                 float eps, float* partial_ws, float* scale, float* shift);
int ffn_gn_apply(void* stream, int dtype, const void* x, void* y, const float* scale, const float* shift, int B, int HW,
                 int C, int silu);
int ffn_groupnorm(void* stream, int dtype, const void* x, void* y, const float* gamma, const float* beta, int B, int HW, int C, int G,
                  float eps, int silu, float* partial_ws, float* scale, float* shift);
int ffn_groupnorm_pair_raw(void* stream, const void* x, void* y_pair, void* yraw_pair, const float* gamma, const float* beta, int B, int HW, int C, int G,
                           float eps, int silu, float* partial_ws, float* scale, float* shift);
int ffn_layernorm(void* stream, int dtype, const void* x, void* y, const float* gamma, const float* beta, int M, int C,
                  float eps);
int ffn_layernorm_pair(void* stream, const float* x, void* y, const float* gamma, const float* beta, int M, int C, float eps);
int ffn_softmax_rows(void* stream, int dtype, const void* x, void* y, long M, int N, float scale);
int ffn_pool_layernorm(void* stream, int dtype, const void* x, const int* ids, void* y, const float* gamma, const float* beta, int N, int S, int C, float eps,
                       int pair);
int ffn_cosine_rows(void* stream, const float* a, const float* b, float* out, int B, int P, int b_rows);

int ffn_cfg_masked(void* stream, const float* eps_u, const float* eps_c, const float* mask, float cfg, float* eps, long n,
                   int HW);
int ffn_ddim_inv_step(void* stream, const float* eps, const float* x, float c_bt, float c_at, float c_an, float c_bn,
                      float* x_next, float* pred_x0, long n);
typedef struct ffn_ctrl_step_desc {
    const float* eps;
    const float* x;
    const float* noise;
    const float* m;
    const float* om;
    float* x_prev;
    float* pred_x0;
    float c_bt, c_at, c_ap, c_dir;
    float c_dirm[8], stdv[8];
    int row_masked[8];
    int rows, CHW, HW;
} ffn_ctrl_step_desc;
int ffn_ddim_ctrl_step(void* stream, const ffn_ctrl_step_desc* d);

typedef struct ffn_pack_desc {
    const float* src;
    void* dst;
    int src_row[16];
    int B, Cl, CP, HW;
} ffn_pack_desc;
int ffn_pack_nchw(void* stream, int dtype, const ffn_pack_desc* d);
int ffn_nhwc_to_nchw_f32(void* stream, const float* src, float* dst, int B, int HW, int C, int ld);
int ffn_concat(void* stream, int dtype, const void* a, const void* b, void* out, long rows, int C1, int C2);
int ffn_timestep_embed(void* stream, int dtype, const float* t_dev, const float* freq, void* out, int B, int half, int flip);
int ffn_transpose(void* stream, int dtype, const void* src, void* dst, int B, int R, int C, int ld_src, int ld_dst);
int ffn_cast(void* stream, int src_dtype, int dst_dtype, const void* src, void* dst, long n);
int ffn_embed_tokens(void* stream, int dtype, const int* ids, const float* table, const float* pos, void* out, long M, int S, int C, int V);
int ffn_image_to_nhwc(void* stream, int dtype, const uint8_t* img, void* dst, long npix, int CP);
int ffn_nhwc_to_image(void* stream, int dtype, const void* src, float* dst, int B, int HW, int ld);

typedef struct ffn_dift_desc {
    const void* src;
    const void* tgt;
    const int* kps;
    void* ws;
    int* out_rc;
    float* out_cos;
    long ws_bytes;
    long es;
    int dtype, E, C, ld, h, w, H, W, K;
} ffn_dift_desc;
int ffn_dift_match(void* stream, const ffn_dift_desc* d);
long ffn_dift_workspace_bytes(int C, int h, int w, int K);

#define FFN_SIFT_MAX_SIDE 16384
#define FFN_SIFT_MAX_TAPS 63
int ffn_sift_base(void* stream, const uint8_t* img, float* out, int H, int W, int C);
int ffn_gauss_blur_f32(void* stream, const float* src, float* dst, float* tmp, int H, int W, const float* taps, int T);
int ffn_decimate2_f32(void* stream, const float* src, float* dst, int H, int W);
int ffn_sift_extrema(void* stream, const float* gauss, float* dog, int h, int w, int* cand, int cap, int* counter, int* count);
int ffn_sift_refine_orient(void* stream, const float* dog, const float* gauss, int h, int w, int octave, const int* cand, int n, float* out);
int ffn_sift_describe(void* stream, const float* gauss, int h, int w, int octave, const float* kp, int n, uint8_t* desc, float* raw);
int ffn_knn2_u8(void* stream, const uint8_t* des1, int n1, const uint8_t* des2, int n2, int* idx, int* dist);

#define FFN_IMGPREP_MAX_SIDE 4096
int ffn_resize_pil_bilinear_u8(void* stream, const uint8_t* src, uint8_t* dst, uint8_t* scratch, int B, int H, int W, int oh, int ow, const int* hbounds,
                               const int* hcoef, int hksize, const int* vbounds, const int* vcoef, int vksize);
int ffn_vit_patch_rows(void* stream, int dtype, const uint8_t* src, const float* lut, void* out, int B, int H, int W, int patch, int ldo);
int ffn_vit_patch_rows_pair(void* stream, const uint8_t* src, const float* lut, void* out, int B, int H, int W, int patch, int K);

#define FFN_IMGPREP_MAX_TAPS (2 * 3 * FFN_IMGPREP_MAX_SIDE + 1)
enum { FFN_KEEP_NONE = 0, FFN_KEEP_SUM_LT128 = 1, FFN_KEEP_GT128 = 2 };
typedef struct {
    const uint8_t* src;
    uint8_t* dst;
    uint8_t* scratch;
    const uint8_t* m1;
    const uint8_t* m2;
    const int* hbounds;
    const int* hcoef;
    const int* vbounds;
    const int* vcoef;
    int B, H, W, C, oh, ow, hksize, vksize;
    int y0, x0, ch, cw;
    int rule;
} ffn_resize_pil_desc;
int ffn_resize_pil_u8(void* stream, const ffn_resize_pil_desc* d);

typedef struct {
    const uint8_t* src_img;
    const uint8_t* src_mask;
    const uint8_t* bg;
    const uint8_t* hole_img;
    const uint8_t* hole_mask;
    const double* inv;
    uint8_t* final_img;
    uint8_t* tmask;
    uint8_t* trans_hole;
    int B, H, W, mask_c, hole_mask_c;
} ffn_coarse_edit_desc;
int ffn_resize_taps8_u8(void* stream, const uint8_t* src, uint8_t* dst, int B, int H, int W, int C, int oh, int ow, const int* iy, const double* wy, const int* ix,
                        const double* wx);
int ffn_resize_gather_u8(void* stream, const uint8_t* src, uint8_t* dst, int B, int H, int W, int C, int oh, int ow, const int* iy, const int* ix, int binarise);
int ffn_dilate_u8(void* stream, const uint8_t* src, uint8_t* dst, uint8_t* scratch, int B, int H, int W, int C, int k);
int ffn_mask_bbox_u8(void* stream, const uint8_t* mask, int* box, int B, int H, int W, int C);
int ffn_coarse_edit_2d(void* stream, const ffn_coarse_edit_desc* d);

int ffn_sam_patch_rows(void* stream, int dtype, const uint8_t* src, void* out, int B, int H, int W, int side, int patch, int ldo, const float* mean, const float* std);
int ffn_sam_patch_rows_pair(void* stream, const uint8_t* src, void* out, int B, int H, int W, int side, int patch, int K, const float* mean, const float* std);
int ffn_hyper_masks(void* stream, const float* up, const float* hyper, float* out, int N, int hw, int C, int M);
int ffn_upsample_bicubic(void* stream, const float* src, float* dst, uint8_t* mask, int N, int h, int w, int H, int W);

#define FFN_BOX_NMS_MAX 16384
int ffn_upsample_bicubic_stats(void* stream, const float* src, int32_t* stats, uint8_t* mask, int N, int h, int w, int H, int W, float offset);
int ffn_box_nms(void* stream, const float* boxes, uint64_t* suppress, int M, float thresh);

// ... 5 lines not shown
```

Before: 2.048.

## Store sub-pixel conv outputs directly to final pixels and merge replay rows into concat buffer

```diff
diff --git a/freefine_amd/_lib.py b/freefine_amd/_lib.py
--- a/freefine_amd/_lib.py
+++ b/freefine_amd/_lib.py
@@ -6,7 +6,7 @@
 
 FFN_F32, FFN_BF16, FFN_BF16X3, FFN_FP8 = 0, 1, 2, 3
 IG_OUT_SILU, IG_OUT_F32, IG_GEGLU, IG_OUT_TRANSPOSED, IG_OUT_PAIR, IG_OUT_GELU, IG_OUT_RELU, IG_OUT_KV64 = 1, 2, 4, 8, 16, 32, 64, 128
-IG_OUT_QGELU = 256
+IG_OUT_QGELU, IG_OUT_UP2X = 256, 512
 ELT_RELU, ELT_ADD, ELT_GELU = 0, 1, 2
 ATT_MAXP, ATT_MAXB = 4, 16
 ATT_HEAD_RULE, ATT_UNIFORM_SEL1, ATT_UNIFORM_SEL0, ATT_CAUSAL = 1, 2, 4, 8
@@ -139,6 +139,7 @@
     "ffn_pack_nchw": (_i, [_vp, _i, C.POINTER(PackDesc)]),
     "ffn_nhwc_to_nchw_f32": (_i, [_vp, _vp, _vp, _i, _i, _i, _i]),
     "ffn_concat": (_i, [_vp, _i, _vp, _vp, _vp, _l, _i, _i]),
+    "ffn_merge_rows": (_i, [_vp, _vp, _i, _l, _vp, _i, _vp, _vp, _i, _l, _i, _l]),
     "ffn_timestep_embed": (_i, [_vp, _i, _vp, _vp, _vp, _i, _i, _i]),
     "ffn_transpose": (_i, [_vp, _i, _vp, _vp, _i, _i, _i, _i, _i]),
     "ffn_cast": (_i, [_vp, _i, _i, _vp, _vp, _l]),
diff --git a/freefine_amd/csrc/capi.hip b/freefine_amd/csrc/capi.hip
--- a/freefine_amd/csrc/capi.hip
+++ b/freefine_amd/csrc/capi.hip
@@ -67,7 +67,7 @@
     return FFN_OK;
 }
 
-extern "C" int ffn_version(void) { return 14; }
+extern "C" int ffn_version(void) { return 15; }
 extern "C" const char* ffn_last_error(void) { return g_err; }
 extern "C" int ffn_device_info(int device, char* name, int name_len) {
     hipDeviceProp_t prop;
@@ -96,7 +96,7 @@
     return n;
 }
 static bool can_split(const ffn_igemm_desc& d) {
-    return d.ws && d.splitk != 1 && !(d.flags & (FFN_IG_GEGLU | FFN_IG_OUT_TRANSPOSED | FFN_IG_OUT_KV64));
+    return d.ws && d.splitk != 1 && !(d.flags & (FFN_IG_GEGLU | FFN_IG_OUT_TRANSPOSED | FFN_IG_OUT_KV64 | FFN_IG_OUT_UP2X));
 }
 static void igemm_rule_for(int dtype, const ffn_igemm_desc& d, int* bm, int* bn, int* splitk) {
     const long t128 = (long)((d.M + 127) / 128) * ((d.N + 127) / 128);
@@ -148,7 +148,7 @@
         if (!can_split(d) || nkt % splitk != 0 || nkt / splitk < 2 || (long)splitk * d.M * d.N * 4 > d.ws_bytes || (long)splitk * d.M * d.N * 4 >= lim) return false;
     } else {
         const int act_ok = (!d.residual && !d.x3 && !d.f8 && !(d.flags & FFN_IG_GEGLU)) ? (FFN_IG_OUT_GELU | FFN_IG_OUT_RELU) : 0;
-        if ((d.alpha != 1.0f && !d.f8) || (d.flags & ~(FFN_IG_GEGLU | act_ok | (d.x3 ? (FFN_IG_OUT_F32 | FFN_IG_OUT_PAIR | FFN_IG_OUT_KV64) : 0)))) return false;
+        if ((d.alpha != 1.0f && !d.f8) || (d.flags & ~(FFN_IG_GEGLU | act_ok | (d.x3 ? (FFN_IG_OUT_F32 | FFN_IG_OUT_PAIR | FFN_IG_OUT_KV64 | (d.conv == 2 ? FFN_IG_OUT_UP2X : 0)) : 0)))) return false;
         if (d.f8 && (!d.conv || (d.flags & FFN_IG_GEGLU))) return false;
         if (d.x3 && (d.flags & FFN_IG_GEGLU) && !(d.flags & FFN_IG_OUT_PAIR)) return false;
         if ((d.flags & FFN_IG_OUT_PAIR) && !(d.flags & FFN_IG_GEGLU) && (d.N % 32 != 0 || (d.ldo / 2) % 32 != 0 || (d.flags & FFN_IG_OUT_TRANSPOSED))) return false;
@@ -171,6 +171,7 @@
         if (a_bytes + 256l * d.lda * 2 >= lim) return false;
     }
     if ((long)d.N * d.Kpad * 2 >= lim || (long)(d.M + 256) * d.ldo * ((d.flags & FFN_IG_OUT_PAIR) ? 2 : osz) >= lim) return false;
+    if ((d.flags & FFN_IG_OUT_UP2X) && (splitk > 1 || 4l * d.M * d.ldo * osz >= lim)) return false;
     if (d.residual && (long)(d.M + 256) * d.ldr * osz >= lim) return false;
     return true;
 }
@@ -402,7 +403,7 @@
     bool f32;
     int bm, bn, amode, nwm, nwn;
     bool swap, fastk, x3, f8;
-    bool res, geglu, split;
+    bool res, geglu, split, up2x;
     int splitk, halo_bytes, lds;
     bool reduce_f32;
     dim3 grid, block;
@@ -458,6 +459,7 @@
         p->split = p->splitk > 1;
         p->res = !p->split && d.residual;
         p->geglu = !p->split && !d.conv && (d.flags & FFN_IG_GEGLU);
+        p->up2x = (d.flags & FFN_IG_OUT_UP2X) != 0;
         [[fallthrough]];
     case IG_PP_TRANS: {
         p->lds = 2 * (p->bm + p->bn) * 128 + 12288;
@@ -502,6 +504,18 @@
 template <int AMODE, bool X3 = false, bool F8 = false>
 static int launch_pp(const IgemmPlan& p, hipStream_t s, const ffn_igemm_desc& d) {
     const bool trans = p.kind == IG_PP_TRANS;
+    if (p.up2x) {
+        if constexpr (X3 && AMODE == AMODE_CONV3) {
+#define FFN_PP_UP2X(BM_, BN_) \
+    if (p.bm == BM_ && p.bn == BN_ && !p.res && !p.split) return igemm_launch(p, igemm_pp_kernel<BM_, BN_, AMODE, false, false, false, false, true, false, true>, s, d, p.splitk)
+            FFN_PP_UP2X(256, 320);
+            FFN_PP_UP2X(256, 256);
+            FFN_PP_UP2X(192, 320);
+            FFN_PP_UP2X(192, 256);
+#undef FFN_PP_UP2X
+        }
+        return fail(FFN_EINVAL, "igemm: no %d x %d ping-pong tile stores to final pixels (FFN_IG_OUT_UP2X)", p.bm, p.bn);
+    }
 #define FFN_PP(BM_, BN_, RES_, GEGLU_, SPLIT_, TRANS_)                                                                       \
     if (p.bm == BM_ && p.bn == BN_ && p.res == RES_ && p.geglu == GEGLU_ && p.split == SPLIT_ && trans == TRANS_) \
         return igemm_launch(p, igemm_pp_kernel<BM_, BN_, AMODE, RES_, GEGLU_, SPLIT_, TRANS_, X3, F8>, s, d, p.splitk)
@@ -648,7 +662,7 @@
         REQUIRE(d.conv && d.Cin > 0 && d.Cin % 16 == 0 && d.K == 9 * d.Cin && d.Kpad >= d.K && d.Kpad % 16 == 0 && d.lda == d.Cin,
                 "igemm(fp8): 3x3 convolutions with Cin %% 16 == 0 only (Cin=%d, K=%d, Kpad=%d, lda=%d)", d.Cin, d.K, d.Kpad, d.lda);
         REQUIRE(d.M > 0 && d.N > 0 && d.N % 4 == 0 && d.ldo % 4 == 0 && d.rows_per_batch > 0 && d.M % (d.Hout * d.Wout) == 0, "igemm(fp8): bad shape");
-        REQUIRE(!(d.flags & (FFN_IG_GEGLU | FFN_IG_OUT_TRANSPOSED | FFN_IG_OUT_PAIR | FFN_IG_OUT_F32)), "igemm(fp8): plain / SiLU / residual epilogues only");
+        REQUIRE(!(d.flags & (FFN_IG_GEGLU | FFN_IG_OUT_TRANSPOSED | FFN_IG_OUT_PAIR | FFN_IG_OUT_F32 | FFN_IG_OUT_UP2X)), "igemm(fp8): plain / SiLU / residual epilogues only");
         REQUIRE(d.stride == 1 || d.stride == 2, "igemm(fp8): stride %d", d.stride);
         int ex = 0;
         REQUIRE(d.alpha > 0.f && frexpf(d.alpha, &ex) == 0.5f, "igemm(fp8): alpha must be a power of two (the un-scaling of two power-of-two operand scales)");
@@ -672,13 +686,19 @@
     }
     REQUIRE(d.K % epc == 0, "igemm: K=%d must be a multiple of %d", d.K, epc);
     REQUIRE(d.rows_per_batch > 0, "igemm: rows_per_batch must be > 0");
+    REQUIRE(!(d.flags & FFN_IG_OUT_UP2X) || d.conv == 2, "igemm: FFN_IG_OUT_UP2X is an output form of conv = 2");
     if (d.conv) {
         REQUIRE(d.Cin % epc == 0, "igemm: Cin=%d must be a multiple of %d", d.Cin, epc);
         if (d.conv == 2) {
             REQUIRE((dtype == FFN_BF16 || dtype == FFN_BF16X3) && d.K == 4 * d.Cin && d.stride == 1 && d.upsample == 0 && d.pad >= 0 && d.pad <= 3 && d.splitk <= 1,
                     "igemm: 2x2 convolution needs FFN_BF16 / FFN_BF16X3, K = 4*Cin, stride 1, no upsample, pad in 0..3, no forced split");
             int bm, bn;
-            REQUIRE(conv2_tile(igemm_view(dtype, d), &bm, &bn), "igemm: 2x2 convolution M=%d N=%d Cin=%d fits no ping-pong tile (Cin %% 64 (split-bf16: 32), N %% 256 / 320, M >= 192)", d.M, d.N, d.Cin);
+            if (d.flags & FFN_IG_OUT_UP2X)
+                REQUIRE(dtype == FFN_BF16X3 && d.Wout > 0 && d.Wout % 16 == 0 && d.Hin == d.Hout && d.Win == d.Wout && !d.residual && !d.rowbias &&
+                            !(d.flags & ~(FFN_IG_OUT_UP2X | FFN_IG_OUT_F32)),
+                        "igemm: FFN_IG_OUT_UP2X needs FFN_BF16X3, Wout %% 16 == 0 (Wout=%d), Hin x Win == Hout x Wout and the bias-only epilogue", d.Wout);
+            REQUIRE(conv2_tile(igemm_view(dtype, d), &bm, &bn), "igemm: 2x2 convolution M=%d N=%d Cin=%d fits no ping-pong tile (Cin %% 64 (split-bf16: 32), N %% 256 / 320, M >= 192%s)", d.M, d.N, d.Cin,
+                    (d.flags & FFN_IG_OUT_UP2X) ? "; FFN_IG_OUT_UP2X: 4 M ldo fp32 below 2 GiB" : "");
         } else {
             REQUIRE(d.conv == 1, "igemm: conv=%d", d.conv);
             REQUIRE(d.K == 9 * d.Cin, "igemm: conv K=%d != 9*Cin=%d", d.K, 9 * d.Cin);
@@ -751,8 +771,8 @@
     case IG_HALO: snprintf(buf, len, "void igemm_halo_kernel<bf16, %d, %d, %d, %d>(ffn_igemm_desc, int)", p.bm, p.bn, p.nwm, p.nwn); break;
     case IG_PP:
     case IG_PP_TRANS:
-        snprintf(buf, len, "void igemm_pp_kernel<%d, %d, %d, %s, %s, %s, %s, %s, %s>(ffn_igemm_desc, int)", p.bm, p.bn, p.amode, b(p.res), b(p.geglu), b(p.split),
-                 b(p.kind == IG_PP_TRANS), b(p.x3), b(p.f8));
+        snprintf(buf, len, "void igemm_pp_kernel<%d, %d, %d, %s, %s, %s, %s, %s, %s%s>(ffn_igemm_desc, int)", p.bm, p.bn, p.amode, b(p.res), b(p.geglu), b(p.split),
+                 b(p.kind == IG_PP_TRANS), b(p.x3), b(p.f8), p.up2x ? ", true" : "");
         break;
     }
     return FFN_OK;
@@ -1618,6 +1638,15 @@
     else LAUNCH(concat_kernel<bf16>, dim3(grid_for(n)), dim3(256), 0, s, (const bf16*)a, (const bf16*)b, (bf16*)out, rows, C1, C2);
     return check_launch("concat");
 }
+extern "C" int ffn_merge_rows(void* stream, const void* a, int n_a, long lda_bytes, const void* r, int n_r, const long* perm, void* out, int n_out, long rows, int row_bytes, long ldo_bytes) {
+    REQUIRE(perm && out && n_a >= 0 && n_r >= 0 && (a || n_a == 0) && (r || n_r == 0) && n_out > 0 && rows > 0, "merge_rows: bad arguments");
+    REQUIRE(row_bytes > 0 && row_bytes % 16 == 0 && ldo_bytes % 16 == 0 && ldo_bytes >= row_bytes && lda_bytes % 16 == 0 && lda_bytes >= row_bytes,
+            "merge_rows: row_bytes=%d, lda_bytes=%ld and ldo_bytes=%ld must be multiples of 16, the strides >= row_bytes", row_bytes, lda_bytes, ldo_bytes);
+    REQUIRE(aligned16(a) && aligned16(r) && aligned16(out), "merge_rows: pointers must be 16-byte aligned");
+    LAUNCH(merge_rows_kernel, dim3(grid_for((long)n_out * rows * (row_bytes / 16))), dim3(256), 0, reinterpret_cast<hipStream_t>(stream), (const u32x4*)a, n_a, lda_bytes / 16, (const u32x4*)r, n_r,
+           perm, (u32x4*)out, n_out, rows, row_bytes / 16, ldo_bytes / 16);
+    return check_launch("merge_rows");
+}
 extern "C" int ffn_timestep_embed(void* stream, int dtype, const float* t_dev, const float* freq, void* out, int B, int half, int flip) {
     REQUIRE(t_dev && freq && out && B > 0 && half > 0, "timestep_embed: bad arguments");
     hipStream_t s = reinterpret_cast<hipStream_t>(stream);
diff --git a/freefine_amd/csrc/elementwise.h b/freefine_amd/csrc/elementwise.h
--- a/freefine_amd/csrc/elementwise.h
+++ b/freefine_amd/csrc/elementwise.h
@@ -80,6 +80,19 @@
         const u32x4 v = (c < c1) ? *reinterpret_cast<const u32x4*>(a + r * C1 + c * EPC)
                                  : *reinterpret_cast<const u32x4*>(b + r * C2 + (c - c1) * EPC);
         *reinterpret_cast<u32x4*>(out + r * (C1 + C2) + c * EPC) = v;
+    }
+}
+
+__global__ __launch_bounds__(256) void merge_rows_kernel(const u32x4* __restrict__ a, int n_a, long lda, const u32x4* __restrict__ r, int n_r, const long* __restrict__ perm,
+                                                         u32x4* __restrict__ out, int n_out, long rows, int cpr, long ldo) {
+    const long per = rows * cpr, n = n_out * per;
+    for (long i = (long)blockIdx.x * 256 + threadIdx.x; i < n; i += (long)gridDim.x * 256) {
+        const long img = i / per, rem = i - img * per;
+        const long row = rem / cpr;
+        const long src = perm[img];
+        if (src < 0 || src >= (long)n_a + n_r) continue;
+        const u32x4 v = src < n_a ? a[(src * rows + row) * lda + (rem - row * cpr)] : r[(src - n_a) * per + rem];
+        out[(img * rows + row) * ldo + (rem - row * cpr)] = v;
     }
 }
 
diff --git a/freefine_amd/csrc/igemm_p8.h b/freefine_amd/csrc/igemm_p8.h
--- a/freefine_amd/csrc/igemm_p8.h
+++ b/freefine_amd/csrc/igemm_p8.h
@@ -36,7 +36,7 @@
 #ifdef PP_TRACE
 __device__ unsigned long long pp_trace[256 * 64];
 #endif
-template <int BM, int BN, int AMODE, bool RES, bool GEGLU, bool SPLIT = false, bool TRANS = false, bool X3 = false, bool F8 = false>
+template <int BM, int BN, int AMODE, bool RES, bool GEGLU, bool SPLIT = false, bool TRANS = false, bool X3 = false, bool F8 = false, bool UP2X = false>
 __global__ __launch_bounds__(512) void igemm_pp_kernel(const IgemmParams p, int splitk = 1) {
     typedef bf16 T;
     constexpr int HM = BM / 2;
@@ -65,6 +65,7 @@
     static_assert(!SPLIT || (!RES && !GEGLU), "split-K slabs carry raw accumulators: the epilogue runs in the reduce kernel");
     static_assert(!TRANS || (!RES && !GEGLU && !SPLIT && AMODE == AMODE_DENSE), "transposed output: dense A, bias only");
     static_assert(!F8 || (!X3 && !TRANS && !GEGLU), "fp8 operands: plain / residual / split-K epilogues");
+    static_assert(!UP2X || (X3 && AMODE == AMODE_CONV3 && !RES && !GEGLU && !SPLIT && !TRANS), "final-pixel stores: split-bf16 sub-pixel convolutions, bias only");
     const int ntn = p.N / BN;
     const int ntm = (p.M + BM - 1) / BM;
     const int nsl = SPLIT ? splitk : 1;
@@ -83,7 +84,8 @@
     const int nbatch = (p.M + p.rows_per_batch - 1) / p.rows_per_batch;
     const __amdgpu_buffer_rsrc_t rsrcRb =
         __builtin_amdgcn_make_buffer_rsrc(const_cast<float*>(p.rowbias), 0, p.rowbias ? ((nbatch - 1) * p.ldrb + p.N) * 4 : 0, 0x00020000);
-    const long o_bytes = TRANS ? (long)((p.M + p.rows_per_batch - 1) / p.rows_per_batch) * p.N * p.ldo * OSZ : (long)p.M * p.ldo * OSZ;
+    const long o_bytes = TRANS ? (long)((p.M + p.rows_per_batch - 1) / p.rows_per_batch) * p.N * p.ldo * OSZ
+                               : (UP2X ? 4l * p.M * p.ldo * OSZ : (long)p.M * p.ldo * OSZ);
     const __amdgpu_buffer_rsrc_t rsrcO = __builtin_amdgcn_make_buffer_rsrc(p.out, 0, (int)o_bytes, 0x00020000);
     const __amdgpu_buffer_rsrc_t rsrcR = __builtin_amdgcn_make_buffer_rsrc(const_cast<void*>(p.residual), 0, RES ? (int)((long)p.M * p.ldr * OSZ) : 0, 0x00020000);
 
@@ -396,10 +398,17 @@
             return;
         }
         if constexpr (X3) {
-            const int voff = (pr * p.ldo + 4 * pg) * 4;
+            const int voff = UP2X ? (pr * 2 * p.ldo + 4 * pg) * 4 : (pr * p.ldo + 4 * pg) * 4;
 #pragma unroll
             for (int i = i0; i < i0 + FH; ++i) {
                 const int vo = m0 + i * 16 + pr < p.M ? voff : OOB;
+                int up_row0 = 0;
+                if constexpr (UP2X) {
+                    const int mf = m0 + i * 16, hw = p.Hout * p.Wout;
+                    const int bi = mf / hw, rem = mf - bi * hw;
+                    const int yy = rem / p.Wout, xx = rem - yy * p.Wout;
+                    up_row0 = ((bi * 2 * p.Hout + 2 * yy + 1 - (p.pad >> 1)) * 2 * p.Wout + 2 * xx + 1 - (p.pad & 1)) * p.ldo;
+                }
                 if constexpr (GEGLU) {
                     const int vo2 = m0 + i * 16 + pr < p.M ? (pr * p.ldo + 4 * pg) * 2 : OOB;
 #pragma unroll
@@ -450,7 +459,8 @@
                             __builtin_amdgcn_raw_buffer_store_b64(lo, rsrcO, vo2, so2 + 128, 0);
                             continue;
                         }
-                        __builtin_amdgcn_raw_buffer_store_b128(w, rsrcO, vo, ((m0 + i * 16) * p.ldo + n0 + j * 16) * 4, 0);
+                        if constexpr (UP2X) __builtin_amdgcn_raw_buffer_store_b128(w, rsrcO, vo, (up_row0 + n0 + j * 16) * 4, 0);
+                        else __builtin_amdgcn_raw_buffer_store_b128(w, rsrcO, vo, ((m0 + i * 16) * p.ldo + n0 + j * 16) * 4, 0);
                     }
                 }
             }
diff --git a/freefine_amd/ops.py b/freefine_amd/ops.py
--- a/freefine_amd/ops.py
+++ b/freefine_amd/ops.py
@@ -80,6 +80,7 @@
 _GN_RAW = os.environ.get("FFN_GN_RAW", "1") != "0"
 _KV64 = os.environ.get("FFN_KV64", "1") != "0"
 _ATTN_PRESPLIT = os.environ.get("FFN_ATTN_PRESPLIT", "1") != "0"
+_DIRECT_OUT = os.environ.get("FFN_DIRECT_OUT", "1") != "0"
 
 
 def _mark_x3(t, order=1):
@@ -170,18 +171,24 @@
     return pack_linear(out.reshape(4 * cout, 4 * cin), dtype)
 
 
-def conv3x3_up2x(x, w4, bias, B, Hin, Win, Cin, *, out=None):
+def conv3x3_up2x(x, w4, bias, B, Hin, Win, Cin, *, out=None, direct=None):
     lib = L.load()
     cout = w4.shape[0] // 4
     x3 = is_x3(w4)
-    per_img = Hin * Win * max(4 * cout * (4 if x3 else 2), Cin * (4 if x3 else 2))
+    if direct is None:
+        direct = _DIRECT_OUT
+    direct = bool(direct) and x3 and Win % 16 == 0
+    if out is not None:
+        assert out.shape == (B, 4 * Hin * Win, cout) and out.stride(-1) == 1 and (B == 1 or out.stride(0) == 4 * Hin * Win * out.stride(-2))
+    ldo = out.stride(-2) if out is not None else cout
+    per_img = Hin * Win * max(4 * (ldo if direct else cout) * (4 if x3 else 2), Cin * (4 if x3 else 2))
     nb = max(1, ((1 << 30) - 1) // per_img)
     if B > nb:
         if out is None:
             out = torch.empty(B, 4 * Hin * Win, cout, dtype=torch.float32 if x3 else x.dtype, device=x.device)
         for b0 in range(0, B, nb):
             b1 = min(B, b0 + nb)
-            conv3x3_up2x(x[b0:b1], w4, bias, b1 - b0, Hin, Win, Cin, out=out[b0:b1])
+            conv3x3_up2x(x[b0:b1], w4, bias, b1 - b0, Hin, Win, Cin, out=out[b0:b1], direct=direct)
         return out
     if x3:
         xa = x if pair_width(x) is not None else split_pair(x, Cin)
@@ -191,7 +198,13 @@
         assert x.dtype == torch.bfloat16 and x.is_contiguous()
         xa, odt, dcode = x, x.dtype, L.FFN_BF16
     assert w4.shape[1] >= (8 if x3 else 4) * Cin
-    y = torch.empty(B, Hin * Win, 4 * cout, dtype=odt, device=x.device)
+    if direct:
+        if out is None:
+            out = torch.empty(B, 4 * Hin * Win, cout, dtype=odt, device=x.device)
+        assert out.dtype == odt
+        y = None
+    else:
+        y = torch.empty(B, Hin * Win, 4 * cout, dtype=odt, device=x.device)
     for c in range(4):
         a, b = c >> 1, c & 1
         d = L.IgemmDesc()
@@ -200,16 +213,21 @@
         d.M, d.N, d.K, d.Kpad = B * Hin * Win, cout, 4 * Cin, w4.stride(0)
         d.lda, d.a_lo, d.x3 = (2 * Cin, 32, 2) if x3 else (Cin, 0, 0)
         d.rows_per_batch, d.ldrb = Hin * Win, 0
-        d.out, d.ldo, d.ldr = y.data_ptr() + c * cout * y.element_size(), 4 * cout, 0
+        if direct:
+            d.out, d.ldo, d.ldr = out.data_ptr(), ldo, 0
+        else:
+            d.out, d.ldo, d.ldr = y.data_ptr() + c * cout * y.element_size(), 4 * cout, 0
         d.Hin, d.Win, d.Cin, d.Hout, d.Wout = Hin, Win, Cin, Hin, Win
         d.stride, d.pad, d.upsample = 1, 2 * (1 - a) + (1 - b), 0
-        d.flags, d.alpha, d.conv = 0, 1.0, 2
+        d.flags, d.alpha, d.conv = (L.IG_OUT_UP2X if direct else 0), 1.0, 2
         d.splitk, d.ws, d.ws_bytes = 0, _workspace(x.device).data_ptr(), WS_BYTES
         if _PROF is None:
             L.check(lib.ffn_igemm(_stream(), dcode, CT.byref(d)), "ffn_igemm(conv 2x2)")
         else:
-            L.check(_timed(_igemm_name(lib, dcode, d), 2.0 * d.M * cout * 4 * Cin, y.element_size() * (x.numel() + cout * 4 * Cin + d.M * cout),
+            L.check(_timed(_igemm_name(lib, dcode, d), 2.0 * d.M * cout * 4 * Cin, (4 if x3 else 2) * (x.numel() + cout * 4 * Cin + d.M * cout),
                            lambda: lib.ffn_igemm(_stream(), dcode, CT.byref(d))), "ffn_igemm(conv 2x2)")
+    if direct:
+        return out
     if out is None:
         out = torch.empty(B, 4 * Hin * Win, cout, dtype=odt, device=x.device)
     out.view(B, Hin, 2, Win, 2, cout).copy_(y.view(B, Hin, Win, 2, 2, cout).permute(0, 1, 3, 2, 4, 5))
@@ -781,6 +799,8 @@
     C1, C2 = a.shape[-1], b.shape[-1]
     rows = a.numel() // C1
     base = getattr(a, "_ffn_cat_base", None)
+    if out is None and base is not None and base.shape[-1] == C1 + C2 and getattr(b, "_ffn_cat_base", None) is base:
+        return base
     if out is None and base is not None and base.shape[-1] == C1 + C2:
         L.check(_timed(f"concat_kernel<{_tname(b)}>", 0.0, 2.0 * rows * C2 * b.element_size(),
                        lambda: lib.ffn_concat(_stream(), _dt(b), None, b.data_ptr(), base.data_ptr(), rows, C1, C2)), "ffn_concat")
@@ -794,9 +814,32 @@
     return out
 
 
+def merge_rows(a, r, perm, out=None):
+    lib = L.load()
+    rowwise = lambda t: t.stride(-1) == 1 and (t.shape[0] == 1 or t.stride(0) == t.shape[1] * t.stride(1))
+    assert a.ndim == 3 and rowwise(a) and r.is_contiguous() and a.shape[1:] == r.shape[1:] and a.dtype == r.dtype
+    assert perm.dtype == torch.int64 and perm.is_contiguous() and perm.device == a.device
+    n, (HW, C) = perm.shape[0], a.shape[1:]
+    if out is None:
+        out = torch.empty(n, HW, C, dtype=a.dtype, device=a.device)
+    assert out.shape == (n, HW, C) and out.dtype == a.dtype and rowwise(out)
+    es = a.element_size()
+    L.check(_timed("merge_rows_kernel", 0.0, 2.0 * n * HW * C * es,
+                   lambda: lib.ffn_merge_rows(_stream(), a.data_ptr(), a.shape[0], a.stride(1) * es, r.data_ptr(), r.shape[0], perm.data_ptr(), out.data_ptr(), n, HW,
+                                              C * es, out.stride(1) * es)), "ffn_merge_rows")
+    return out
+
+
 def cat_dst(shape_lead, C1, C2, dtype, device):
     base = torch.empty(*shape_lead, C1 + C2, dtype=dtype, device=device)
     view = base[..., :C1]
+    view._ffn_cat_base = base
+    return view
+
+
+def cat_right(left):
+    base = left._ffn_cat_base
+    view = base[..., left.shape[-1]:]
     view._ffn_cat_base = base
     return view
 
diff --git a/freefine_amd/unet.py b/freefine_amd/unet.py
--- a/freefine_amd/unet.py
+++ b/freefine_amd/unet.py
@@ -681,10 +681,17 @@
                 if replay:
                     state = ru.get("state_run") or ru["state"]
                     assert len(state) == 1 + len(skips), (len(state), len(skips))
-                    merge = lambda a, r: torch.cat([a, r.to(a.dtype)], 0).index_select(0, ru["perm"])
-                    x = merge(x, state[0])
-                    skips = [(merge(s, st), sh, sw) for (s, sh, sw), st in zip(skips, reversed(state[1:]))]
                     B, temb_all = BB, temb_full
+                    if ops._DIRECT_OUT and skips and all(t.shape[-1] * t.element_size() % 16 == 0 for t in [x] + [s for s, _, _ in skips]):
+                        merge = lambda a, r, out=None: ops.merge_rows(a, r.to(a.dtype).contiguous(), ru["perm"], out=out)
+                        xd = cat_dst(x.shape[-1], x.shape[1])
+                        x = merge(x, state[0], xd)
+                        top = merge(skips[-1][0], state[1], ops.cat_right(xd))
+                        skips = [(merge(s, st), sh, sw) for (s, sh, sw), st in zip(skips[:-1], list(reversed(state[1:]))[:-1])] + [(top,) + skips[-1][1:]]
+                    else:
+                        merge = lambda a, r: torch.cat([a, r.to(a.dtype)], 0).index_select(0, ru["perm"])
+                        x = merge(x, state[0])
+                        skips = [(merge(s, st), sh, sw) for (s, sh, sw), st in zip(skips, reversed(state[1:]))]
                     self._in_phase_a = False
             for j, r in enumerate(blk.res):
                 s, sh, sw = skips.pop()
diff --git a/include/freefine_hip.h b/include/freefine_hip.h
--- a/include/freefine_hip.h
+++ b/include/freefine_hip.h
@@ -23,7 +23,8 @@
     FFN_IG_OUT_GELU = 1 << 5,
     FFN_IG_OUT_KV64 = 1 << 7,
     FFN_IG_OUT_RELU = 1 << 6,
-    FFN_IG_OUT_QGELU = 1 << 8
+    FFN_IG_OUT_QGELU = 1 << 8,
+    FFN_IG_OUT_UP2X = 1 << 9
 };
 typedef struct ffn_igemm_desc {
     const void* A;
@@ -163,6 +164,7 @@
 int ffn_pack_nchw(void* stream, int dtype, const ffn_pack_desc* d);
 int ffn_nhwc_to_nchw_f32(void* stream, const float* src, float* dst, int B, int HW, int C, int ld);
 int ffn_concat(void* stream, int dtype, const void* a, const void* b, void* out, long rows, int C1, int C2);
+int ffn_merge_rows(void* stream, const void* a, int n_a, long lda_bytes, const void* r, int n_r, const long* perm, void* out, int n_out, long rows, int row_bytes, long ldo_bytes);
 int ffn_timestep_embed(void* stream, int dtype, const float* t_dev, const float* freq, void* out, int B, int half, int flip);
 int ffn_transpose(void* stream, int dtype, const void* src, void* dst, int B, int R, int C, int ld_src, int ld_dst);
 int ffn_cast(void* stream, int src_dtype, int dst_dtype, const void* src, void* dst, long n);
```

After: 2.061 (median of 6 runs). About the same (+0.6%).
